# facebookresearch/DRTK

Measured on AMD Instinct MI355X. Metric: Mpixels/sec fwd+bwd, 100k-tri @ 2048x2048, 1/2/4/8 GPU; HBM BW %, higher is better.
Workload: dtype f32; 1 GPU; 8 views/GPU x 1 GPU, 100k-tri UV-sphere head mesh (F=100352, V=50400), 2048x2048, C=16 attribute channels, transform+rasterize+render+interpolate+mask+edge_grad_estimator+loss fwd+bwd; views_per_gpu=8, triangles=100352, vertices=50400, height=2048, width=2048, channels=16, grad_reset=set_to_none, parallelism=single GPU

## Files before the change

drtk_amd/capi.py:

```python
import ctypes
import os
from typing import Optional, Tuple

import torch as th

from drtk_amd.utils import native_library_paths

_lib = None

DRTK_F32, DRTK_F64 = 0, 1


_lib_path = None

_POISON = os.environ.get("DRTK_CAPI_POISON", "") not in ("", "0")


_GUARD = int(os.environ.get("DRTK_CAPI_GUARD", "0") or 0)
_guards = []


def _sentinel(dtype):
    return 0x5A if dtype == th.uint8 else (-7.25 if dtype.is_floating_point else -(2 ** 29) - 3)


def _out(*shape, dtype, device):
    if _GUARD:
        n = 1
        for d in shape:
            n *= int(d)
        g = _GUARD * (16 if dtype == th.uint8 else 1)
        flat = th.full((n + 2 * g,), _sentinel(dtype), dtype=dtype, device=device)
        _guards.append((flat, g, n))
        t = flat[g:g + n].view(*shape)
    else:
        t = th.empty(*shape, dtype=dtype, device=device)
    if _POISON and t.numel():
        if t.dtype.is_floating_point:
            t.fill_(float("nan"))
        elif t.dtype == th.uint8:
            t.fill_(0xA5)
        else:
            t.fill_(-(2 ** 30) - 7)
    return t


def check_guards() -> int:
    th.cuda.synchronize()
    k = len(_guards)
    for flat, g, n in _guards:
        s = _sentinel(flat.dtype)
        ok = bool((flat[:g] == s).all()) and bool((flat[g + n:] == s).all())
        if not ok:
            _guards.clear()
            raise AssertionError(f"a kernel wrote outside a {flat.dtype} output / workspace of {n} elements")
    _guards.clear()
    return k



def use_profiling_library(path: str) -> None:
    global _lib_path
    assert _lib is None, "the C-ABI library is already loaded"
    _lib_path = path


DEPTH_ORDERS = {"strict": 0, "fastmath": 1}


def use_depth_order(order: str) -> None:
    assert order in DEPTH_ORDERS, order
    _check(lib().drtk_amd_set_depth_order(DEPTH_ORDERS[order]), "set_depth_order")


def depth_order() -> str:
    o = lib().drtk_amd_get_depth_order()
    return next(k for k, v in DEPTH_ORDERS.items() if v == o)


def lib() -> ctypes.CDLL:
    global _lib
    if _lib is None:
        path = _lib_path or native_library_paths()[0]
        if not os.path.isfile(path):
            build_py = os.path.join(os.path.dirname(os.path.abspath(__file__)), "build.py")
            raise ImportError(f"{path} is missing: run `python {build_py}`")
        L = ctypes.CDLL(path)
        L.drtk_amd_status_string.restype = ctypes.c_char_p
        L.drtk_amd_status_string.argtypes = [ctypes.c_int]
        L.drtk_amd_version.restype = ctypes.c_char_p
        for name in EXPORTS:
            if name not in ("drtk_amd_status_string", "drtk_amd_version"):
                getattr(L, name).restype = ctypes.c_int
        _lib = L
    return _lib


EXPORTS = [
    "drtk_amd_status_string",
    "drtk_amd_version",
    "drtk_amd_set_depth_order",
    "drtk_amd_get_depth_order",
    "drtk_amd_rasterize_workspace_bytes",
    "drtk_amd_rasterize_lines_workspace_bytes",
    "drtk_amd_rasterize",
    "drtk_amd_rasterize_layers_workspace_bytes",
    "drtk_amd_rasterize_layers",
    "drtk_amd_render",
    "drtk_amd_render_backward",
    "drtk_amd_interpolate",
    "drtk_amd_interpolate_masked",
    "drtk_amd_interpolate_backward",
    "drtk_amd_interpolate_backward_workspace_bytes",
    "drtk_amd_interpolate_backward_ws",
    "drtk_amd_edge_grad_backward_workspace_bytes",
    "drtk_amd_edge_grad_backward",
    "drtk_amd_edge_grad_backward_fused_workspace_bytes",
    "drtk_amd_edge_grad_backward_fused",
    "drtk_amd_interpolation_matrix",
    "drtk_amd_interpolation_matrix_backward",
    "drtk_amd_interpolation_normal_matrix_values",
    "drtk_amd_interpolation_normal_matrix_values_backward",
    "drtk_amd_mipmap_grid_sampler_2d",
    "drtk_amd_mipmap_grid_sampler_2d_backward",
    "drtk_amd_grid_scatter_2d",
    "drtk_amd_grid_scatter_2d_backward",
    "drtk_amd_screen_space_uv_derivative",
    "drtk_amd_transform_pinhole",
    "drtk_amd_transform_pinhole_backward",
    "drtk_amd_geometry_face_forward",
    "drtk_amd_geometry_face_backward",
    "drtk_amd_geometry_face_gather",
    "drtk_amd_geometry_vertex_gather_workspace_bytes",
    "drtk_amd_geometry_vertex_gather",
    "drtk_amd_selftest_exact_div",
    "drtk_amd_kernel_timing_begin",
    "drtk_amd_kernel_timing_report",
]


class DrtkAmdError(RuntimeError):
    pass


def _check(status: int, what: str):
    if status != 0:
        raise DrtkAmdError(f"{what}: {lib().drtk_amd_status_string(status).decode()} (status {status})")


def _dt(t: th.Tensor) -> int:
    if t.dtype == th.float32:
        return DRTK_F32
    if t.dtype == th.float64:
        return DRTK_F64
    raise TypeError(f"drtk_amd: unsupported dtype {t.dtype}")


def _p(t: Optional[th.Tensor]):
    return ctypes.c_void_p(0 if t is None else t.data_ptr())


def _i(x) -> ctypes.c_int64:
    return ctypes.c_int64(int(x))


def _on_tensor_device(fn):
    import functools

    def tensors(args):
        for a in args:
            if isinstance(a, th.Tensor):
                yield a
            elif isinstance(a, (list, tuple)):
                yield from (x for x in a if isinstance(x, th.Tensor))

    @functools.wraps(fn)
    def guarded(*args, **kwargs):
        ts = list(tensors(list(args) + list(kwargs.values())))
        if not ts:
            return fn(*args, **kwargs)
        if not ts[0].is_cuda:
            raise DrtkAmdError("drtk_amd implements the MI355X (HIP) path only; got a CPU tensor")
        devs = {t.device for t in ts}
        if len(devs) != 1:
            raise DrtkAmdError(f"drtk_amd: tensors of one call on different devices: {sorted(map(str, devs))}")
        with th.cuda.device(ts[0].device):
            return fn(*args, **kwargs)

    return guarded


def _stream(t: th.Tensor, stream) -> ctypes.c_void_p:
    if not t.is_cuda:
        raise DrtkAmdError("drtk_amd implements the MI355X (HIP) path only; got a CPU tensor")
    s = th.cuda.current_stream(t.device) if stream is None else stream
    return ctypes.c_void_p(s.cuda_stream)


def _vi(vi: th.Tensor, n: int):
    assert vi.dtype == th.int32
    if vi.ndim == 2:
        c = vi.contiguous()
        return c, 0, c.shape[0]
    if vi.shape[0] > 1 and vi.stride(0) == 0:
        c = vi[0].contiguous()
        return c, 0, c.shape[0]
    c = vi.contiguous()
    return c, c.shape[1] * 3, c.shape[1]


def rasterize_workspace_bytes(N, F, H, W) -> int:
    out = ctypes.c_size_t(0)
    _check(lib().drtk_amd_rasterize_workspace_bytes(_i(N), _i(F), _i(H), _i(W), ctypes.byref(out)), "rasterize")
    return out.value


def rasterize_lines_workspace_bytes(N, H, W) -> int:
    out = ctypes.c_size_t(0)
    _check(lib().drtk_amd_rasterize_lines_workspace_bytes(_i(N), _i(H), _i(W), ctypes.byref(out)), "rasterize")
    return out.value


@_on_tensor_device
def rasterize(v, vi, height, width, stream=None, workspace=None, wireframe=False, out=None) -> Tuple[th.Tensor, th.Tensor]:
    v = v.contiguous()
    N, V, _ = v.shape
    vi_c, vi_sN, F = _vi(vi, N)
    if out is not None:
        depth, index = out
        assert depth.shape == (N, height, width) and index.shape == (N, height, width) and depth.is_contiguous() and index.is_contiguous()
        assert depth.dtype == th.float32 and index.dtype == th.int32
    else:
        depth = _out(N, height, width, dtype=th.float32, device=v.device)
        index = _out(N, height, width, dtype=th.int32, device=v.device)
    nbytes = rasterize_lines_workspace_bytes(N, height, width) if wireframe else rasterize_workspace_bytes(N, F, height, width)
    ws = workspace if workspace is not None else _out(nbytes, dtype=th.uint8, device=v.device)
    _check(
        lib().drtk_amd_rasterize(
            ctypes.c_int(_dt(v)), _p(v), _p(vi_c), _i(N), _i(V), _i(F), _i(vi_sN), _i(height), _i(width),
            ctypes.c_int(1 if wireframe else 0), _p(depth), _p(index), _p(ws), ctypes.c_size_t(ws.numel()),
            _stream(v, stream)),
        "rasterize")
    return depth, index


MAX_RASTER_LAYERS = 8


def rasterize_layers_workspace_bytes(N, F, H, W, num_layers) -> int:
    out = ctypes.c_size_t(0)
    _check(
        lib().drtk_amd_rasterize_layers_workspace_bytes(_i(N), _i(F), _i(H), _i(W), ctypes.c_int(int(num_layers)), ctypes.byref(out)),
        "rasterize_layers")
    return out.value


@_on_tensor_device
def rasterize_layers(v, vi, height, width, num_layers, stream=None, workspace=None, out=None) -> Tuple[th.Tensor, th.Tensor]:
    v = v.contiguous()
    N, V, _ = v.shape
    K = int(num_layers)
    vi_c, vi_sN, F = _vi(vi, N)
    nbytes = rasterize_layers_workspace_bytes(N, F, height, width, K)
    if out is not None:
        depth, index = out
        assert depth.shape == (N, K, height, width) and index.shape == (N, K, height, width) and depth.is_contiguous() and index.is_contiguous()
        assert depth.dtype == th.float32 and index.dtype == th.int32
    else:
        depth = _out(N, K, height, width, dtype=th.float32, device=v.device)
        index = _out(N, K, height, width, dtype=th.int32, device=v.device)
    ws = workspace if workspace is not None else _out(nbytes, dtype=th.uint8, device=v.device)
    _check(
        lib().drtk_amd_rasterize_layers(
            ctypes.c_int(_dt(v)), _p(v), _p(vi_c), _i(N), _i(V), _i(F), _i(vi_sN), _i(height), _i(width),
            ctypes.c_int(K), _p(depth), _p(index), _p(ws), ctypes.c_size_t(ws.numel()), _stream(v, stream)),
        "rasterize_layers")
    return depth, index


@_on_tensor_device
def render(v, vi, index_img, stream=None):
    v = v.contiguous()
    index_img = index_img.contiguous()
    N, V, _ = v.shape
    H, W = index_img.shape[1:]
    vi_c, vi_sN, F = _vi(vi, N)
    depth = _out(N, H, W, dtype=v.dtype, device=v.device)
    bary = _out(N, 3, H, W, dtype=v.dtype, device=v.device)
    _check(
        lib().drtk_amd_render(
            ctypes.c_int(_dt(v)), _p(v), _p(vi_c), _p(index_img), _i(N), _i(V), _i(F), _i(vi_sN), _i(H), _i(W),
            _p(depth), _p(bary), _stream(v, stream)),
        "render")
    return depth, bary


@_on_tensor_device
def render_backward(v, vi, index_img, grad_depth_img, grad_bary_img, stream=None):
    v = v.contiguous()
    index_img = index_img.contiguous()
    gd, gb = grad_depth_img.contiguous(), grad_bary_img.contiguous()
    N, V, _ = v.shape
    H, W = index_img.shape[1:]
    vi_c, vi_sN, F = _vi(vi, N)
    grad_v = _out(N, V, 3, dtype=v.dtype, device=v.device)
    _check(
        lib().drtk_amd_render_backward(
            ctypes.c_int(_dt(v)), _p(v), _p(vi_c), _p(index_img), _p(gd), _p(gb), _i(N), _i(V), _i(F), _i(vi_sN),
            _i(H), _i(W), _p(grad_v), _stream(v, stream)),
        "render_backward")
    return grad_v


@_on_tensor_device
def interpolate(attrs, vi, index_img, bary_img, stream=None, masked=False):
    attrs = attrs.contiguous()
    index_img = index_img.contiguous()
    bary_img = bary_img.contiguous()
    N, V, C = attrs.shape
    H, W = index_img.shape[1:]
    vi_c, vi_sN, F = _vi(vi, N)
    out = _out(N, C, H, W, dtype=attrs.dtype, device=attrs.device)
    fn = lib().drtk_amd_interpolate_masked if masked else lib().drtk_amd_interpolate
    _check(
        fn(ctypes.c_int(_dt(attrs)), _p(attrs), _p(vi_c), _p(index_img), _p(bary_img), _i(N), _i(V), _i(C), _i(F),
           _i(vi_sN), _i(H), _i(W), _p(out), _stream(attrs, stream)),
        "interpolate_masked" if masked else "interpolate")
    return out


def interpolate_masked(attrs, vi, index_img, bary_img, stream=None):
    return interpolate(attrs, vi, index_img, bary_img, stream, masked=True)


@_on_tensor_device
def interpolate_backward(grad_out, attrs, vi, index_img, bary_img, vert_requires_grad=True,
                         bary_requires_grad=True, stream=None, workspace=None):
    grad_out = grad_out.contiguous()
    attrs = attrs.contiguous()
    index_img = index_img.contiguous()
    bary_img = bary_img.contiguous()
    N, V, C = attrs.shape
    H, W = index_img.shape[1:]
    vi_c, vi_sN, F = _vi(vi, N)
    ag = _out(N, V, C, dtype=attrs.dtype, device=attrs.device) if vert_requires_grad else None
    bg = _out(N, 3, H, W, dtype=attrs.dtype, device=attrs.device) if bary_requires_grad else None
    ws, nbytes = None, 0
    if os.environ.get("DRTK_CAPI_NO_INTERP_WS"):
        workspace = False
    if vert_requires_grad and workspace is not False:
        out = ctypes.c_size_t(0)
        _check(lib().drtk_amd_interpolate_backward_workspace_bytes(ctypes.c_int(_dt(attrs)), _i(N), _i(V), _i(C), ctypes.byref(out)), "interpolate_backward")
        nbytes = int(out.value)
        if nbytes:
            ws = _out((nbytes + 3) // 4, dtype=th.float32, device=attrs.device)
            assert ws.data_ptr() % 64 == 0 or os.environ.get("DRTK_CAPI_GUARD"), "torch allocations are 256-byte aligned"
            if ws.data_ptr() % 64 != 0:
                ws, nbytes = None, 0
    _check(
        lib().drtk_amd_interpolate_backward_ws(
            ctypes.c_int(_dt(attrs)), _p(grad_out), _p(attrs), _p(vi_c), _p(index_img), _p(bary_img), _i(N), _i(V),
            _i(C), _i(F), _i(vi_sN), _i(H), _i(W), _p(ag), _p(bg), _p(ws), ctypes.c_size_t(nbytes), _stream(attrs, stream)),
        "interpolate_backward")
    return ag, bg


@_on_tensor_device
def interpolation_matrix(vi, index_img, bary_img, stream=None):
    index_img = index_img.contiguous()
    bary_img = bary_img.contiguous()
    N, H, W = index_img.shape
    vi_c, vi_sN, F = _vi(vi, N)
    row_pixels = th.nonzero(index_img.reshape(-1).ne(-1)).reshape(-1)
    R = row_pixels.numel()
    crow = th.arange(0, 3 * R + 1, 3, dtype=th.int64, device=index_img.device)
    col = _out(3 * R, dtype=th.int64, device=index_img.device)
    values = _out(3 * R, dtype=bary_img.dtype, device=bary_img.device)
    _check(
        lib().drtk_amd_interpolation_matrix(
            ctypes.c_int(_dt(bary_img)), _p(vi_c), _p(index_img), _p(bary_img), _p(row_pixels), _i(R), _i(N), _i(F),
            _i(vi_sN), _i(H), _i(W), _p(col), _p(values), _stream(bary_img, stream)),
        "interpolation_matrix")
    return crow, col, values, row_pixels


@_on_tensor_device
def interpolation_matrix_backward(grad_values, vi, index_img, row_pixels, stream=None):
    grad_values = grad_values.contiguous()
    index_img = index_img.contiguous()
    row_pixels = row_pixels.contiguous()
    N, H, W = index_img.shape
    vi_c, vi_sN, F = _vi(vi, N)
    bg = _out(N, 3, H, W, dtype=grad_values.dtype, device=grad_values.device)
    _check(
        lib().drtk_amd_interpolation_matrix_backward(
            ctypes.c_int(_dt(grad_values)), _p(grad_values), _p(vi_c), _p(index_img), _p(row_pixels),
            _i(row_pixels.numel()), _i(N), _i(F), _i(vi_sN), _i(H), _i(W), _p(bg), _stream(grad_values, stream)),
        "interpolation_matrix_backward")
    return bg


def _pairs(pair_indices, N):
    assert pair_indices.dtype == th.int32 and pair_indices.shape[-1] == 9
    if pair_indices.ndim == 2:
        return pair_indices.contiguous(), 0, pair_indices.shape[0]
    if pair_indices.shape[0] == N and N > 1 and pair_indices.stride(0) == 0:
        return pair_indices[0].contiguous(), 0, pair_indices.shape[1]
    p = pair_indices.contiguous()
    return p, p.shape[1] * 9, p.shape[1]


@_on_tensor_device
def interpolation_normal_matrix_values(pair_indices, index_img, bary_img, nnz, stream=None):
    index_img = index_img.contiguous()
    bary_img = bary_img.contiguous()
    N, H, W = index_img.shape
    pr, pair_sN, F = _pairs(pair_indices, N)
    values = _out(nnz, dtype=bary_img.dtype, device=bary_img.device)
    _check(
        lib().drtk_amd_interpolation_normal_matrix_values(
            ctypes.c_int(_dt(bary_img)), _p(pr), _p(index_img), _p(bary_img), _i(N), _i(F), _i(pair_sN), _i(H), _i(W),
            _i(nnz), _p(values), _stream(bary_img, stream)),
        "interpolation_normal_matrix_values")
    return values


@_on_tensor_device
def interpolation_normal_matrix_values_backward(grad_values, pair_indices, index_img, bary_img, stream=None):
    grad_values = grad_values.contiguous()
    index_img = index_img.contiguous()
    bary_img = bary_img.contiguous()
    N, H, W = index_img.shape
    pr, pair_sN, F = _pairs(pair_indices, N)
    bg = _out(N, 3, H, W, dtype=bary_img.dtype, device=bary_img.device)
    _check(
        lib().drtk_amd_interpolation_normal_matrix_values_backward(
            ctypes.c_int(_dt(bary_img)), _p(grad_values), _p(pr), _p(index_img), _p(bary_img), _i(N), _i(F),
            _i(pair_sN), _i(H), _i(W), _p(bg), _stream(bary_img, stream)),
        "interpolation_normal_matrix_values_backward")
    return bg


def _level_table(levels):
    lv = []
    for t in levels:
        ok = t.dim() == 4 and (t.shape[0] == 0 or t[0].is_contiguous()) and (t.stride(0) == 0 or t.stride(0) >= t[0].numel() or t.shape[0] <= 1)
        lv.append(t if ok else t.contiguous())
    n = len(lv)
    ptrs = (ctypes.c_void_p * n)(*[t.data_ptr() for t in lv])
    lh = (ctypes.c_int64 * n)(*[t.shape[2] for t in lv])
    lw = (ctypes.c_int64 * n)(*[t.shape[3] for t in lv])
    lsn = (ctypes.c_int64 * n)(*[(t.stride(0) if t.shape[0] > 1 else t.shape[1] * t.shape[2] * t.shape[3]) for t in lv])
    return lv, ptrs, lh, lw, lsn


def _grid_layout(grid):
    N, H, W, two = grid.shape
    sN, sH, sW, sC = grid.stride()
    P = H * W
    rows_ok = H <= 1 or sH == W * sW
    pixel_major = sC == 1 and sW == 2 and rows_ok and (N <= 1 or sN >= 2 * P)
    channel_major = sW == 1 and sC >= P and rows_ok and (N <= 1 or sN >= sC + P)
    if not (two == 2 and P > 0 and (pixel_major or channel_major)):
        grid = grid.contiguous()
        sN, sW, sC = 2 * P, 2, 1
    return grid, (ctypes.c_int64 * 3)(sN if N > 1 else 2 * P, sW, sC)


@_on_tensor_device
def mipmap_grid_sampler_2d(levels, grid, vt_dxdy_img, max_aniso, padding_mode=0, interpolation_mode=0,
                           align_corners=False, force_max_aniso=False, clip_grad=False, stream=None):
    lv, ptrs, lh, lw, lsn = _level_table(levels)
    grid, glayout = _grid_layout(grid)
    vt = vt_dxdy_img.contiguous()
    N, C = lv[0].shape[:2]
    H, W = grid.shape[1:3]
    out = _out(N, C, H, W, dtype=lv[0].dtype, device=lv[0].device)
    _check(
        lib().drtk_amd_mipmap_grid_sampler_2d(
            ctypes.c_int(_dt(lv[0])), ptrs, lh, lw, lsn, ctypes.c_int(len(lv)), _p(grid), glayout, _p(vt), _i(N), _i(C), _i(H), _i(W),
            ctypes.c_int(max_aniso), ctypes.c_int(padding_mode), ctypes.c_int(interpolation_mode),
            ctypes.c_int(bool(align_corners)), ctypes.c_int(bool(force_max_aniso)), ctypes.c_int(bool(clip_grad)),
            _p(out), _stream(lv[0], stream)),
        "mipmap_grid_sampler_2d")
    return out


@_on_tensor_device
def mipmap_grid_sampler_2d_backward(grad_out, levels, grid, vt_dxdy_img, max_aniso, padding_mode=0,
                                    interpolation_mode=0, align_corners=False, force_max_aniso=False,
                                    clip_grad=False, stream=None):
    lv, ptrs, lh, lw, lsn = _level_table(levels)
    grid, glayout = _grid_layout(grid)
    vt = vt_dxdy_img.contiguous()
    grad_out = grad_out.contiguous()
    N, C = lv[0].shape[:2]
    H, W = grid.shape[1:3]
    flat = _out(sum(t.numel() for t in lv), dtype=lv[0].dtype, device=lv[0].device)
    glv, off = [], 0
    for t in lv:
        glv.append(flat[off:off + t.numel()].view(t.shape))
        off += t.numel()
    gptrs = (ctypes.c_void_p * len(lv))(*[t.data_ptr() for t in glv])
    ggrid = th.empty_strided(grid.shape, grid.stride(), dtype=grid.dtype, device=grid.device)
    _check(
        lib().drtk_amd_mipmap_grid_sampler_2d_backward(
            ctypes.c_int(_dt(lv[0])), _p(grad_out), ptrs, lh, lw, lsn, ctypes.c_int(len(lv)), _p(grid), glayout, _p(vt), _i(N), _i(C),
            _i(H), _i(W), ctypes.c_int(max_aniso), ctypes.c_int(padding_mode), ctypes.c_int(interpolation_mode),
            ctypes.c_int(bool(align_corners)), ctypes.c_int(bool(force_max_aniso)), ctypes.c_int(bool(clip_grad)),
            gptrs, _p(ggrid), glayout, _stream(lv[0], stream)),
        "mipmap_grid_sampler_2d_backward")
    return glv, ggrid


@_on_tensor_device
def grid_scatter_2d(input, grid, output_height, output_width, padding_mode=1, interpolation_mode=0, align_corners=False,
                    stream=None, route_counts=None):
    input = input.contiguous()
    grid, glayout = _grid_layout(grid)
    N, C, H, W = input.shape
    assert grid.shape == (N, H, W, 2) and grid.dtype == input.dtype, (grid.shape, input.shape)
    if route_counts is not None:
        assert route_counts.numel() == 2 and route_counts.element_size() == 4 and route_counts.is_contiguous() and route_counts.device == input.device
    out = _out(N, C, int(output_height), int(output_width), dtype=input.dtype, device=input.device)
    _check(
        lib().drtk_amd_grid_scatter_2d(
            ctypes.c_int(_dt(input)), _p(input), _p(grid), glayout, _i(N), _i(C), _i(H), _i(W), _i(output_height),
            _i(output_width), ctypes.c_int(padding_mode), ctypes.c_int(interpolation_mode), ctypes.c_int(bool(align_corners)),
            _p(out), _p(route_counts), _stream(input, stream)),
        "grid_scatter_2d")
    return out


@_on_tensor_device
def grid_scatter_2d_backward(grad_out, input, grid, padding_mode=1, interpolation_mode=0, align_corners=False,
                             input_requires_grad=True, grid_requires_grad=True, stream=None):
    input = input.contiguous()
    grad_out = grad_out.contiguous()
    grid, glayout = _grid_layout(grid)
    N, C, H, W = input.shape
    OH, OW = grad_out.shape[2:]
    assert grad_out.shape[:2] == (N, C) and grid.shape == (N, H, W, 2)
    gi = _out(N, C, H, W, dtype=input.dtype, device=input.device) if input_requires_grad else None
    gg = None
    if grid_requires_grad:
        gg = th.empty_strided(grid.shape, grid.stride(), dtype=grid.dtype, device=grid.device)
        if _POISON and gg.numel():
            gg.fill_(float("nan"))
    _check(
        lib().drtk_amd_grid_scatter_2d_backward(
            ctypes.c_int(_dt(input)), _p(grad_out), _p(input), _p(grid), glayout, _i(N), _i(C), _i(H), _i(W), _i(OH), _i(OW),
            ctypes.c_int(padding_mode), ctypes.c_int(interpolation_mode), ctypes.c_int(bool(align_corners)), _p(gi), _p(gg),
            glayout, _stream(input, stream)),
        "grid_scatter_2d_backward")
    return gi, gg


@_on_tensor_device
def screen_space_uv_derivative(v, vt, vi, vti, index_img, bary_img, mask, campos, camrot, focal, stream=None):
    index_img = index_img.contiguous()
    bary_img = bary_img.contiguous()
    N, H, W = index_img.shape
    v_c, vt_c = v.contiguous(), vt.contiguous()
    v_sN = 0 if v_c.ndim == 2 else v_c.shape[1] * 3
    vt_sN = 0 if vt_c.ndim == 2 else vt_c.shape[1] * 2
    V, T = v_c.shape[-2], vt_c.shape[-2]
    vi_c, vti_c = vi.contiguous(), vti.contiguous()
    m = None if mask is None else mask.to(th.uint8).contiguous()
    out = _out(N, H, W, 2, 2, dtype=bary_img.dtype, device=bary_img.device)
    _check(
        lib().drtk_amd_screen_space_uv_derivative(
            ctypes.c_int(_dt(bary_img)), _p(v_c), _i(v_sN), _p(vt_c), _i(vt_sN), _p(vi_c), _p(vti_c), _p(index_img),
            _p(bary_img), _p(m), _p(campos.contiguous()), _p(camrot.contiguous()), _p(focal.contiguous()), _i(N), _i(V),
            _i(T), _i(vi_c.shape[0]), _i(H), _i(W), _p(out), _stream(bary_img, stream)),
        "screen_space_uv_derivative")
    return out


GEOMETRY_CHUNK = 256


def vertex_incidence_numpy(vi, num_vertices: int, chunk: int = GEOMETRY_CHUNK):
    import numpy as np

    t = np.asarray(vi, dtype=np.int64)
    t = t[None] if t.ndim == 2 else t
    B, F = t.shape[0], t.shape[1]
    V = int(num_vertices)
    keys = (t + (np.arange(B, dtype=np.int64) * V)[:, None, None]).reshape(-1)
    perm = np.argsort(keys, kind="stable")
    entries = (perm % max(3 * F, 1)).astype(np.int32)
    crow = np.searchsorted(keys[perm], np.arange(B * V + 1), side="left").astype(np.int64)
    length = np.diff(crow)
    nch = np.where(length > chunk, (length + chunk - 1) // chunk, 0)
    chunk_ptr = np.concatenate([[0], np.cumsum(nch)]).astype(np.int64)
    chunk_row = np.repeat(np.arange(B * V), nch)
    chunk_begin = crow[chunk_row] + (np.arange(len(chunk_row)) - chunk_ptr[chunk_row]) * chunk
    return tuple(a.astype(np.int32) for a in (crow, entries, chunk_ptr, chunk_begin, chunk_row))


def _geometry_topology(vi: th.Tensor):
    assert vi.dtype == th.int32
    c = vi.contiguous()
    if c.ndim == 2 or c.shape[0] == 1:
        return c, 0, 1
    return c, c.shape[1] * 3, c.shape[0]


@_on_tensor_device
def geometry_face_forward(v, vi, vt=None, vti=None, outputs=("normals", "areas", "edges"), stream=None):
    v = v.contiguous()
    N, V = v.shape[0], v.shape[1]
    vi_c, vi_sN, _ = _geometry_topology(vi)
    F = vi_c.shape[-2]
    shapes = {"normals": (N, F, 3), "areas": (N, F, 1), "edges": (N, F, 3, 3), "dpdt": (N, F, 2, 3),
              "dpdt_u": (N, F, 3), "v012": (N, F, 3, 3)}
    out = {k: _out(*shapes[k], dtype=v.dtype, device=v.device) for k in outputs}
    vt_c = None if vt is None else vt.contiguous()
    vti_c = None if vti is None else vti.contiguous()
    T = 0 if vt_c is None else vt_c.shape[1]
    _check(
        lib().drtk_amd_geometry_face_forward(
            ctypes.c_int(_dt(v)), _p(v), _i(V * 3), _p(vi_c), _i(vi_sN), _p(vt_c), _i(T * 2), _p(vti_c), _i(N), _i(V),
            _i(T), _i(F), *(_p(out.get(k)) for k in ("normals", "areas", "edges", "dpdt", "dpdt_u", "v012")),
            _stream(v, stream)),
        "geometry_face_forward")
    return out


@_on_tensor_device
def geometry_face_backward(v, vi, vt=None, vti=None, grad_vert=None, vert_sums=None, grad_normals=None,
                           grad_areas=None, grad_edges=None, grad_dpdt=None, grad_v012=None, stream=None):
    v = v.contiguous()
    N, V = v.shape[0], v.shape[1]
    vi_c, vi_sN, _ = _geometry_topology(vi)
    F = vi_c.shape[-2]
    vt_c = None if vt is None else vt.contiguous()
    vti_c = None if vti is None else vti.contiguous()
    T = 0 if vt_c is None else vt_c.shape[1]
    pos = _out(N, F, 3, 3, dtype=v.dtype, device=v.device)
    uv = None if vt_c is None else _out(N, F, 3, 2, dtype=v.dtype, device=v.device)
    c = [None if g is None else g.contiguous() for g in (grad_vert, vert_sums, grad_normals, grad_areas, grad_edges,
                                                          grad_dpdt, grad_v012)]
    _check(
        lib().drtk_amd_geometry_face_backward(
            ctypes.c_int(_dt(v)), _p(v), _i(V * 3), _p(vi_c), _i(vi_sN), _p(vt_c), _i(T * 2), _p(vti_c), _i(N), _i(V),
            _i(T), _i(F), *(_p(g) for g in c), _p(pos), _p(uv), _stream(v, stream)),
        "geometry_face_backward")
    return pos, uv


@_on_tensor_device
def geometry_face_gather(grad_vert, vi, num_faces=None, vert_sums=None, stream=None):
    g = grad_vert.contiguous()
    N, V, A = g.shape
    vi_c, vi_sN, _ = _geometry_topology(vi)
    F = vi_c.shape[-2]
    out = _out(N, F, A, dtype=g.dtype, device=g.device)
    s = None if vert_sums is None else vert_sums.contiguous()
    _check(lib().drtk_amd_geometry_face_gather(ctypes.c_int(_dt(g)), _p(g), _p(s), _p(vi_c), _i(vi_sN), _i(N), _i(V),
                                               _i(F), _i(A), _p(out), _stream(g, stream)),
           "geometry_face_gather")
    return out


@_on_tensor_device
def geometry_vertex_gather(src, incidence, num_vertices, per_corner=False, normalize=False, stream=None):
    src = src.contiguous()
    N, F, A = src.shape[0], src.shape[1], src.shape[-1]
    inc = [th.as_tensor(a, dtype=th.int32, device=src.device).contiguous() for a in incidence]
    crow, entries, chunk_ptr, chunk_begin, chunk_row = inc
    V = int(num_vertices)
    B = (crow.numel() - 1) // V if V else 1
    C = chunk_row.numel()
    out = _out(N, V, A, dtype=src.dtype, device=src.device)
    sums = _out(N, V, 3, dtype=src.dtype, device=src.device) if normalize else None
    need = ctypes.c_size_t(0)
    _check(lib().drtk_amd_geometry_vertex_gather_workspace_bytes(ctypes.c_int(_dt(src)), _i(N), _i(B), _i(C), _i(A),
                                                                 ctypes.byref(need)), "geometry_vertex_gather")
    ws = _out(max(need.value, 1), dtype=th.uint8, device=src.device)
    _check(
        lib().drtk_amd_geometry_vertex_gather(
            ctypes.c_int(_dt(src)), _p(src), _i(F * A * (3 if per_corner else 1)), ctypes.c_int(int(bool(per_corner))),
            _i(A), _p(crow), _p(entries), _p(chunk_ptr if C else None), _p(chunk_begin if C else None),
            _p(chunk_row if C else None), _i(C), _i(B), _i(N), _i(V), _i(F), ctypes.c_int(int(bool(normalize))), _p(out),
            _p(sums), _p(ws), ctypes.c_size_t(need.value), _stream(src, stream)),
        "geometry_vertex_gather")
    return out, sums


def edge_grad_backward_workspace_bytes(dtype, N, H, W) -> int:
    out = ctypes.c_size_t(0)
    code = DRTK_F32 if dtype == th.float32 else DRTK_F64
    _check(lib().drtk_amd_edge_grad_backward_workspace_bytes(ctypes.c_int(code), _i(N), _i(H), _i(W), ctypes.byref(out)),
           "edge_grad_backward")
    return out.value


@_on_tensor_device
def edge_grad_backward(v_pix, img, index_img, vi, grad_output, max_dp_dr=1e4, stream=None, workspace=None):
    v_pix = v_pix.contiguous()
    img = img.contiguous()
    index_img = index_img.contiguous()
    grad_output = grad_output.contiguous()
    N, V, _ = v_pix.shape
    C, H, W = img.shape[1:]
    vi_c, vi_sN, F = _vi(vi, N)
    out = _out(N, 3, H, W, dtype=v_pix.dtype, device=v_pix.device)
    nbytes = edge_grad_backward_workspace_bytes(v_pix.dtype, N, H, W)
    ws = workspace if workspace is not None else _out(nbytes, dtype=th.uint8, device=v_pix.device)
    _check(
        lib().drtk_amd_edge_grad_backward(
            ctypes.c_int(_dt(v_pix)), _p(v_pix), _p(img), _p(index_img), _p(vi_c), _p(grad_output), _i(N), _i(V),
            _i(C), _i(F), _i(vi_sN), _i(H), _i(W), ctypes.c_double(max_dp_dr), _p(out), _p(ws),
            ctypes.c_size_t(ws.numel()), _stream(v_pix, stream)),
        "edge_grad_backward")
    return out


@_on_tensor_device
def edge_grad_backward_fused(v_pix, img, index_img, vi, bary_img, grad_output, max_dp_dr=1e4, stream=None):
    v_pix = v_pix.contiguous()
    img = img.contiguous()
    index_img = index_img.contiguous()
    bary_img = bary_img.contiguous()
    grad_output = grad_output.contiguous()
    N, V, _ = v_pix.shape
    C, H, W = img.shape[1:]
    vi_c, vi_sN, F = _vi(vi, N)
    out = _out(N, V, 3, dtype=v_pix.dtype, device=v_pix.device)
    nb = ctypes.c_size_t(0)
    code = DRTK_F32 if v_pix.dtype == th.float32 else DRTK_F64
    _check(lib().drtk_amd_edge_grad_backward_fused_workspace_bytes(ctypes.c_int(code), _i(N), _i(H), _i(W), ctypes.byref(nb)),
           "edge_grad_backward_fused")
    ws = _out(nb.value, dtype=th.uint8, device=v_pix.device)
    _check(
        lib().drtk_amd_edge_grad_backward_fused(
            ctypes.c_int(_dt(v_pix)), _p(v_pix), _p(img), _p(index_img), _p(vi_c), _p(bary_img), _p(grad_output),
            _i(N), _i(V), _i(C), _i(F), _i(vi_sN), _i(H), _i(W), ctypes.c_double(max_dp_dr), _p(out), _p(ws),
            ctypes.c_size_t(ws.numel()), _stream(v_pix, stream)),
        "edge_grad_backward_fused")
    return out


def selftest_exact_div(dtype=th.float32, seed=1, count=1 << 28, device="cuda:0") -> int:
    out = th.zeros(1, dtype=th.int64, device=device)
    code = DRTK_F32 if dtype == th.float32 else DRTK_F64
    _check(lib().drtk_amd_selftest_exact_div(ctypes.c_int(code), ctypes.c_uint64(seed), _i(count), _p(out),
                                             _stream(out, None)), "selftest_exact_div")
    return int(out.item())


def kernel_timing_begin() -> None:
    _check(lib().drtk_amd_kernel_timing_begin(), "kernel_timing_begin")


def kernel_timing_report() -> dict:
    need = ctypes.c_size_t(0)
    buf = ctypes.create_string_buffer(1 << 16)
    _check(lib().drtk_amd_kernel_timing_report(buf, ctypes.c_size_t(len(buf)), ctypes.byref(need)), "kernel_timing_report")
    out = {}
    for line in buf.value.decode().splitlines():
        name, count, ms = line.rsplit("\t", 2)
        out[name.strip("()")] = (int(count), float(ms))
    return out
```

drtk_amd/csrc/rasterize.hip:

```cpp
#include <algorithm>

#include "common.hpp"
#include "segscatter.hpp"

#ifdef DRTK_AMD_ABLATION
namespace drtk_amd {
__device__ unsigned long long g_phase_clocks[16];
}
extern "C" __attribute__((visibility("default"))) int drtk_amd_debug_read_phases(unsigned long long* out) {
  if (hipDeviceSynchronize() != hipSuccess) return DRTK_ERR_LAUNCH;
  if (hipMemcpyFromSymbol(out, HIP_SYMBOL(drtk_amd::g_phase_clocks), 16 * sizeof(unsigned long long)) != hipSuccess) return DRTK_ERR_LAUNCH;
  const unsigned long long zero[16] = {};
  if (hipMemcpyToSymbol(HIP_SYMBOL(drtk_amd::g_phase_clocks), zero, sizeof(zero)) != hipSuccess) return DRTK_ERR_LAUNCH;
  return DRTK_OK;
}
#define DRTK_PHASE_INIT() unsigned long long drtk_phase_t_ = __builtin_readcyclecounter()
#define DRTK_PHASE(i)                                                     \
  do {                                                                    \
    if (DRTK_DBG(dbg, 256)) {  \
      const unsigned long long now_ = __builtin_readcyclecounter();       \
      atomicAdd(&::drtk_amd::g_phase_clocks[i], now_ - drtk_phase_t_);    \
      drtk_phase_t_ = __builtin_readcyclecounter();                       \
    }                                                                     \
  } while (0)
#else
#define DRTK_PHASE_INIT() do { } while (0)
#define DRTK_PHASE(i) do { } while (0)
#endif

namespace drtk_amd {
namespace {

constexpr uint32_t kCulled = 0xFFFFFFFFu;
constexpr uint32_t kFacingBit = 0x80000000u;
constexpr int kMaxSmallTiles = 4;

template <typename T>
struct TriSetup {
  T p0x, p0y, p1x, p1y, p2x, p2y;
  T dinv0, dinv1, dinv2;
  T sign_denom, abs_denom, rdenom;
  int bb_min_x, bb_min_y, bb_max_x, bb_max_y;
  bool c0, c1, c2;
  bool tl0, tl1, tl2;
  uint32_t z_lo_bits;
};

template <typename T>
struct DivRange;
template <>
struct DivRange<float> {
  static __device__ constexpr float lo() { return 0x1p-60f; }
  static __device__ constexpr float hi() { return 0x1p60f; }
  static __device__ constexpr float tiny() { return 0x1p-100f; }
};
template <>
struct DivRange<double> {
  static __device__ constexpr double lo() { return 0x1p-500; }
  static __device__ constexpr double hi() { return 0x1p500; }
  static __device__ constexpr double tiny() { return 0x1p-900; }
};
__device__ __forceinline__ float fma_t(float a, float b, float c) {
  return __builtin_fmaf(a, b, c);
}
__device__ __forceinline__ double fma_t(double a, double b, double c) {
  return __builtin_fma(a, b, c);
}
template <typename T>
__device__ __forceinline__ bool exact_div_ok(T d) {
  return d >= DivRange<T>::lo() && d <= DivRange<T>::hi();
}
template <typename T>
__device__ __forceinline__ T exact_div(T n, T d, T r, bool range_ok) {
  const T q0 = n * r;
  if (range_ok && (q0 >= DivRange<T>::tiny() || n == T(0))) {
    const T q1 = fma_t(fma_t(-d, q0, n), r, q0);
    return fma_t(fma_t(-d, q1, n), r, q1);
  }
  return n / d;
}

template <typename T>
__device__ __forceinline__ T markstein2(T n, T d, T r, T q0) {
  const T q1 = fma_t(fma_t(-d, q0, n), r, q0);
  return fma_t(fma_t(-d, q1, n), r, q1);
}

__device__ __forceinline__ float exact_rcp(float x) {
  const uint32_t bits = __float_as_uint(x);
  const float ax = __uint_as_float(bits & 0x7FFFFFFFu);
  if ((bits & 0x7FFFFFu) != 0x7FFFFFu && ax >= 0x1p-100f && ax <= 0x1p100f) {
    const float y = __builtin_amdgcn_rcpf(x);
    return __builtin_fmaf(y, __builtin_fmaf(-x, y, 1.0f), y);
  }
  return 1.0f / x;
}
__device__ __forceinline__ double exact_rcp(double x) {
  return 1.0 / x;
}
__device__ __forceinline__ bool fast_rcp_ok(float x) {
  const uint32_t bits = __float_as_uint(x);
  const float ax = __uint_as_float(bits & 0x7FFFFFFFu);
  return ((bits & 0x7FFFFFu) != 0x7FFFFFu) & (ax >= 0x1p-100f) & (ax <= 0x1p100f);
}
__device__ __forceinline__ float fast_rcp(float x) {
  const float y = __builtin_amdgcn_rcpf(x);
  return __builtin_fmaf(y, __builtin_fmaf(-x, y, 1.0f), y);
}
__device__ __forceinline__ bool fast_rcp_ok(double) {
  return true;
}
__device__ __forceinline__ bool fast_rcp_ok_clamped(float x) {
  const uint32_t bits = __float_as_uint(x);
  return ((bits & 0x7FFFFFu) != 0x7FFFFFu) & (__uint_as_float(bits & 0x7FFFFFFFu) <= 0x1p100f);
}
__device__ __forceinline__ bool fast_rcp_ok_clamped(double) {
  return true;
}
template <typename T>
__device__ __forceinline__ T smallest_positive_if(bool on);
template <>
__device__ __forceinline__ float smallest_positive_if<float>(bool on) {
  return __uint_as_float(on ? 1u : 0u);
}
template <>
__device__ __forceinline__ double smallest_positive_if<double>(bool on) {
  return __longlong_as_double(on ? 1ll : 0ll);
}
__device__ __forceinline__ double fast_rcp(double x) {
  return 1.0 / x;
}

template <typename T>
__device__ __forceinline__ uint32_t z_lower_bound_bits(T min_x, T max_x, T min_y, T max_y, T abs_denom, T zmin) {
  const T ext = (max_x - min_x > max_y - min_y ? max_x - min_x : max_y - min_y) + T(2);
  const T eps = sizeof(T) == 4 ? T(5.97e-8) : T(1.12e-16);
  const T delta = T(40) * eps * ext * ext / abs_denom + T(2e-6);
  if (!(delta < T(0.25))) return 0u;
  const T cap = (T(1) / Eps<T>::value()) * (T(1) - T(2e-6));
  const T zb = zmin * (T(1) - delta);
  const float lo = static_cast<float>(zb < cap ? zb : cap);
  const uint32_t bits = __float_as_uint(lo);
  return (lo > 0.0f && bits > 8u) ? bits - 8u : 0u;
}

template <typename T>
__device__ __forceinline__ uint32_t z_upper_bound_bits(const TriSetup<T>& s) {
  const T min_x = min3(s.p0x, s.p1x, s.p2x), min_y = min3(s.p0y, s.p1y, s.p2y);
  const T max_x = max3(s.p0x, s.p1x, s.p2x), max_y = max3(s.p0y, s.p1y, s.p2y);
  const T ext = (max_x - min_x > max_y - min_y ? max_x - min_x : max_y - min_y) + T(2);
  const T eps = sizeof(T) == 4 ? T(5.97e-8) : T(1.12e-16);
  const T delta = T(40) * eps * ext * ext / s.abs_denom + T(2e-6);
  if (!(delta < T(0.25))) return 0xFFFFFFFFu;
  const T zb = (T(1) / min3(s.dinv0, s.dinv1, s.dinv2)) / (T(1) - delta);
  const float hi = static_cast<float>(zb);
  if (!(hi > 0.0f && hi < 1e30f)) return 0xFFFFFFFFu;
  return __float_as_uint(hi) + 8u;
}

template <typename T>
__device__ __forceinline__ bool tri_bbox(
    const T* __restrict__ v_n, const int32_t* __restrict__ vi_face, int H, int W, int& bx0,
    int& by0, int& bx1, int& by1, bool& positive, float& z_mean, uint32_t& z_lo_bits) {
  const int32_t vi_0 = static_cast<int32_t>(static_cast<uint32_t>(vi_face[0]) & 0x0FFFFFFFu);
  const int32_t vi_1 = vi_face[1];
  const int32_t vi_2 = vi_face[2];
  if (vi_0 == vi_1 && vi_1 == vi_2) return false;
  const T p0x = v_n[3 * (int64_t)vi_0 + 0], p0y = v_n[3 * (int64_t)vi_0 + 1], p0z = v_n[3 * (int64_t)vi_0 + 2];
  const T p1x = v_n[3 * (int64_t)vi_1 + 0], p1y = v_n[3 * (int64_t)vi_1 + 1], p1z = v_n[3 * (int64_t)vi_1 + 2];
  const T p2x = v_n[3 * (int64_t)vi_2 + 0], p2y = v_n[3 * (int64_t)vi_2 + 1], p2z = v_n[3 * (int64_t)vi_2 + 2];
  if (!(p0z > T(1e-8f) && p1z > T(1e-8f) && p2z > T(1e-8f))) return false;
  const T min_x = min3(p0x, p1x, p2x), min_y = min3(p0y, p1y, p2y);
  const T max_x = max3(p0x, p1x, p2x), max_y = max3(p0y, p1y, p2y);
  if (!(min_x <= T(W - 1) && min_y <= T(H - 1) && max_x > T(0) && max_y > T(0))) return false;
  const T v01x = p1x - p0x, v01y = p1y - p0y, v02x = p2x - p0x, v02y = p2y - p0y;
  const T den = v01x * v02y - v01y * v02x;
  if (den == T(0)) return false;
  positive = den > T(0);
  z_lo_bits = z_lower_bound_bits<T>(min_x, max_x, min_y, max_y, den > T(0) ? den : -den, min3(p0z, p1z, p2z));
  z_mean = static_cast<float>((p0z + p1z + p2z) * T(1.0 / 3.0));
  bx0 = max(0, trunc_i32(min_x));
  by0 = max(0, trunc_i32(min_y));
  bx1 = min(W - 1, static_cast<int32_t>(static_cast<uint32_t>(trunc_i32(max_x)) + 1u));
  by1 = min(H - 1, static_cast<int32_t>(static_cast<uint32_t>(trunc_i32(max_y)) + 1u));
  return bx0 <= bx1 && by0 <= by1;
}

template <typename T>
__device__ __forceinline__ bool tri_setup(
    const T* __restrict__ v_n, const int32_t* __restrict__ vi_face, int H, int W, TriSetup<T>& s) {
  const int32_t vi_0 = static_cast<int32_t>(static_cast<uint32_t>(vi_face[0]) & 0x0FFFFFFFu);
  const int32_t vi_1 = vi_face[1];
  const int32_t vi_2 = vi_face[2];
  if (vi_0 == vi_1 && vi_1 == vi_2) return false;
  s.p0x = v_n[3 * (int64_t)vi_0 + 0];
  s.p0y = v_n[3 * (int64_t)vi_0 + 1];
  s.p1x = v_n[3 * (int64_t)vi_1 + 0];
  s.p1y = v_n[3 * (int64_t)vi_1 + 1];
  s.p2x = v_n[3 * (int64_t)vi_2 + 0];
  s.p2y = v_n[3 * (int64_t)vi_2 + 1];
  const T p0z = v_n[3 * (int64_t)vi_0 + 2];
  const T p1z = v_n[3 * (int64_t)vi_1 + 2];
  const T p2z = v_n[3 * (int64_t)vi_2 + 2];
  if (!(p0z > T(1e-8f) && p1z > T(1e-8f) && p2z > T(1e-8f))) return false;
  const T min_x = min3(s.p0x, s.p1x, s.p2x), min_y = min3(s.p0y, s.p1y, s.p2y);
  const T max_x = max3(s.p0x, s.p1x, s.p2x), max_y = max3(s.p0y, s.p1y, s.p2y);
  if (!(min_x <= T(W - 1) && min_y <= T(H - 1) && max_x > T(0) && max_y > T(0))) return false;
  const T v01x = s.p1x - s.p0x, v01y = s.p1y - s.p0y;
  const T v02x = s.p2x - s.p0x, v02y = s.p2y - s.p0y;
  const T v12x = s.p2x - s.p1x, v12y = s.p2y - s.p1y;
  const T den = v01x * v02y - v01y * v02x;
  if (den == T(0)) return false;
  s.sign_denom = den > T(0) ? T(1) : T(-1);
  s.abs_denom = den > T(0) ? den : -den;
  s.rdenom = T(1) / s.abs_denom;
  s.bb_min_x = max(0, trunc_i32(min_x));
  s.bb_min_y = max(0, trunc_i32(min_y));
  s.bb_max_x = min(W - 1, static_cast<int32_t>(static_cast<uint32_t>(trunc_i32(max_x)) + 1u));
  s.bb_max_y = min(H - 1, static_cast<int32_t>(static_cast<uint32_t>(trunc_i32(max_y)) + 1u));
  s.dinv0 = T(1) / epsclamp(p0z);
  s.dinv1 = T(1) / epsclamp(p1z);
  s.dinv2 = T(1) / epsclamp(p2z);
  s.c0 = vi_1 <= vi_2;
  s.c1 = vi_2 <= vi_0;
  s.c2 = vi_0 <= vi_1;
  const bool pos = den > T(0);
  s.tl0 = pos ? (v12y < T(0) || (v12y == T(0) && v12x > T(0))) : (v12y > T(0) || (v12y == T(0) && v12x < T(0)));
  s.tl1 = pos ? (v02y > T(0) || (v02y == T(0) && v02x < T(0))) : (v02y < T(0) || (v02y == T(0) && v02x > T(0)));
  s.tl2 = pos ? (v01y < T(0) || (v01y == T(0) && v01x > T(0))) : (v01y > T(0) || (v01y == T(0) && v01x < T(0)));
  s.z_lo_bits = 0;
  return true;
}

template <typename T>
__device__ __forceinline__ T edge_fn(T ax, T ay, T bx, T by, T px, T py) {
  return (py - ay) * (bx - ax) - (px - ax) * (by - ay);
}
template <typename T>
__device__ __forceinline__ T canon_edge(bool a_le_b, T ax, T ay, T bx, T by, T px, T py) {
  return a_le_b ? edge_fn(ax, ay, bx, by, px, py) : -edge_fn(bx, by, ax, ay, px, py);
}

template <typename T>
__device__ __forceinline__ bool fragment(const TriSetup<T>& s, int x, int y, uint32_t& depth_bits) {
  const T px = static_cast<T>(x), py = static_cast<T>(y);
  T b0 = canon_edge(s.c0, s.p1x, s.p1y, s.p2x, s.p2y, px, py) * s.sign_denom;
  T b1 = canon_edge(s.c1, s.p2x, s.p2y, s.p0x, s.p0y, px, py) * s.sign_denom;
  T b2 = canon_edge(s.c2, s.p0x, s.p0y, s.p1x, s.p1y, px, py) * s.sign_denom;
  if (!((b0 >= T(0)) && (b1 >= T(0)) && (b2 >= T(0)))) return false;
  if ((!s.tl0 && b0 == T(0)) || (!s.tl1 && b1 == T(0)) || (!s.tl2 && b2 == T(0))) return false;
  b0 /= s.abs_denom;
  b1 /= s.abs_denom;
  b2 /= s.abs_denom;
  const T depth_inverse = s.dinv0 * b0 + s.dinv1 * b1 + s.dinv2 * b2;
  const float depth = static_cast<float>(T(1) / epsclamp(depth_inverse));
  depth_bits = __float_as_uint(depth);
  return true;
}

#ifndef DRTK_RASTER_QUEUE_SHARDS
#define DRTK_RASTER_QUEUE_SHARDS 8
#endif
constexpr int kQueueShards = DRTK_RASTER_QUEUE_SHARDS;
constexpr int kQueueStride = 32;
constexpr uint32_t kItemEmpty = 0x80000000u;

struct BinLayout {
  int tile_shift;
  int tiles_x, tiles_y;
  int64_t tiles_per_view, num_tiles;
  size_t off_count, off_cursor, off_big_count, off_view_stats, off_queue, zero_bytes;
  size_t off_offset, off_range, off_pre, off_big_list, off_pairs, off_items, total_bytes;
  int64_t max_items;
};

constexpr int kSplit4Min = 384, kSplit4Max = 2048;
inline int split_threshold(int64_t N, int64_t F) {
#ifndef DRTK_RASTER_SPLIT_SLOTS
#define DRTK_RASTER_SPLIT_SLOTS 4
#endif
  const int64_t slots = int64_t(num_compute_units()) * DRTK_RASTER_SPLIT_SLOTS;
  const int64_t t = (N * F * 13) / (20 * (slots > 0 ? slots : 1));
  return static_cast<int>(t < kSplit4Min ? kSplit4Min : (t > kSplit4Max ? kSplit4Max : t));
}
__host__ __device__ inline uint32_t make_item(uint32_t tile, uint32_t sub, uint32_t split_log) {
  return tile | (sub << 24) | (split_log << 28);
}

inline size_t align_up(size_t x, size_t a) {
  return (x + a - 1) / a * a;
}

inline BinLayout make_layout(int64_t N, int64_t F, int64_t H, int64_t W) {
  BinLayout L;
  const int64_t t64 = N * ceil_div(W, 64) * ceil_div(H, 64);
  L.tile_shift = (t64 >= 2048) ? 6 : 5;
  const int64_t ts = int64_t(1) << L.tile_shift;
  L.tiles_x = static_cast<int>(ceil_div(W, ts));
  L.tiles_y = static_cast<int>(ceil_div(H, ts));
  L.tiles_per_view = int64_t(L.tiles_x) * L.tiles_y;
  L.num_tiles = N * L.tiles_per_view;
  size_t o = 0;
  L.off_count = o;
  o += align_up(sizeof(unsigned long long) * L.num_tiles, 256);
  L.off_cursor = o;
  o += align_up(sizeof(unsigned long long) * L.num_tiles, 256);
  L.off_big_count = o;
  o += align_up(sizeof(int32_t) * (N > 0 ? N : 1), 256);
  L.off_view_stats = o;
  o += align_up(sizeof(float) * 4 * (N > 0 ? N : 1), 256);
  L.off_queue = o;
  o += align_up(sizeof(int32_t) * kQueueStride * (1 + kQueueShards), 256);
  L.zero_bytes = o;
  L.off_offset = o;
  o += align_up(sizeof(int32_t) * (L.num_tiles + 1), 256);
  L.off_range = o;
  o += align_up(sizeof(uint2) * N * F, 256);
  L.off_pre = o;
  o += align_up(sizeof(uint4) * N * F, 256);
  L.off_big_list = o;
  o += align_up(sizeof(int32_t) * N * F, 256);
  L.off_pairs = o;
  o += align_up(sizeof(int32_t) * kMaxSmallTiles * N * F, 256);
  L.max_items = L.num_tiles + 16 * ((kMaxSmallTiles * N * F) / kSplit4Min);
  L.off_items = o;
  o += align_up(sizeof(uint32_t) * L.max_items, 256);
  L.total_bytes = o > 0 ? o : 256;
  return L;
}

template <bool BOTH, bool FETCH>
__device__ __forceinline__ int wave_agg_inc2(unsigned long long* __restrict__ counters, int key, bool on, bool hi) {
  const int lane = lane_id();
  unsigned long long todo = __ballot(on);
  int pos = 0;
  while (todo) {
    const int leader = __builtin_amdgcn_readfirstlane(__builtin_ctzll(todo));
    const int k = __builtin_amdgcn_readlane(key, leader);
    const bool mine = on && key == k;
    const unsigned long long same = __ballot(mine);
    const unsigned long long same_hi = __ballot(mine && hi);
    const unsigned long long same_lo = BOTH ? same : (same & ~same_hi);
    unsigned long long base = 0;
    if (lane == leader) {
      const unsigned long long add =
          static_cast<unsigned long long>(__popcll(same_lo)) | (static_cast<unsigned long long>(__popcll(same_hi)) << 32);
      if (FETCH) {
        base = atomicAdd(counters + k, add);
      } else {
        atomicAdd(counters + k, add);
      }
    }
    if (FETCH) {
      const unsigned lo = __builtin_amdgcn_readlane(static_cast<int>(base & 0xFFFFFFFFull), leader);
      const unsigned hh = __builtin_amdgcn_readlane(static_cast<int>(base >> 32), leader);
      const unsigned long long below = (1ull << lane) - 1ull;
      if (mine) pos = hi ? static_cast<int>(hh) + __popcll(same_hi & below) : static_cast<int>(lo) + __popcll(same_lo & below);
    }
    todo &= ~same;
  }
  return pos;
}

template <typename T>
__global__ __launch_bounds__(kBlock) void bin_count_kernel(
    const T* __restrict__ v, const int32_t* __restrict__ vi, int F, int64_t V, int64_t vi_sN, int H,
    int W, int tile_shift, int tiles_x, int tiles_per_view, unsigned long long* __restrict__ tile_count,
    int32_t* __restrict__ big_count, int32_t* __restrict__ big_list,
    uint2* __restrict__ tri_range, uint4* __restrict__ tri_pre, float* __restrict__ view_stats) {
  const int n = blockIdx.y;
  const int f = blockIdx.x * kBlock + threadIdx.x;
  const bool in_range = f < F;
  int bx0, by0, bx1, by1;
  uint2 r = make_uint2(kCulled, kCulled);
  int tx0 = 0, ty0 = 0, tw = 0, ntiles = 0;
  bool positive = false;
  float z_mean = 0.0f;
  uint32_t z_lo_bits = 0;
  if (in_range &&
      tri_bbox<T>(v + int64_t(n) * V * 3, vi + int64_t(n) * vi_sN + int64_t(f) * 3, H, W, bx0, by0, bx1, by1, positive, z_mean, z_lo_bits)) {
    const bool fits = bx1 < 65536 && by1 < 65536;
    tri_pre[int64_t(n) * F + f] = make_uint4(
        static_cast<uint32_t>(bx0) | (static_cast<uint32_t>(bx1) << 16), static_cast<uint32_t>(by0) | (static_cast<uint32_t>(by1) << 16),
        fits ? z_lo_bits : 0u, fits ? 1u : 0u);
    tx0 = bx0 >> tile_shift;
    ty0 = by0 >> tile_shift;
    const int tx1 = bx1 >> tile_shift, ty1 = by1 >> tile_shift;
    r.x = static_cast<uint32_t>(tx0) | (static_cast<uint32_t>(tx1) << 16);
    r.y = static_cast<uint32_t>(ty0) | (static_cast<uint32_t>(ty1) << 16) | (positive ? kFacingBit : 0u);
    tw = tx1 - tx0 + 1;
    ntiles = tw * (ty1 - ty0 + 1);
  }
  if ((blockIdx.x & 63) == 0) {
    const bool live = ntiles >= 1;
    float zp = (live && positive) ? z_mean : 0.0f, zn = (live && !positive) ? z_mean : 0.0f;
#pragma unroll
    for (int o = 32; o > 0; o >>= 1) {
      zp += __shfl_xor(zp, o);
      zn += __shfl_xor(zn, o);
    }
    const int cp = __popcll(__ballot(live && positive)), cn = __popcll(__ballot(live && !positive));
    if (lane_id() == 0 && (cp | cn)) {
      float* st = view_stats + 4 * n;
      if (cp) {
        atomic_add_global(st + 0, zp);
        atomic_add_global(st + 1, static_cast<float>(cp));
      }
      if (cn) {
        atomic_add_global(st + 2, zn);
        atomic_add_global(st + 3, static_cast<float>(cn));
      }
    }
  }
  if (in_range) tri_range[int64_t(n) * F + f] = r;
  const bool small = ntiles >= 1 && ntiles <= kMaxSmallTiles;
  const int base = n * tiles_per_view;
  for (int s = 0; s < kMaxSmallTiles; ++s) {
    const bool on = small && s < ntiles;
    const int dy = on ? s / tw : 0;
    const int dx = on ? s - dy * tw : 0;
    const int t = base + (ty0 + dy) * tiles_x + tx0 + dx;
    wave_agg_inc2<true, false>(tile_count, t, on, positive);
  }
  const bool big = ntiles > kMaxSmallTiles;
  if (__ballot(big)) {
    const int pos = wave_agg_inc<true>(big_count, n, big);
    if (big) big_list[int64_t(n) * F + pos] = f;
  }
}

__global__ __launch_bounds__(1024) void bin_scan_kernel(
    const unsigned long long* __restrict__ tile_count64, int32_t* __restrict__ tile_offset, int num_tiles,
    int tile_shift, int split4, uint32_t* __restrict__ items, int32_t* __restrict__ queue) {
  constexpr int kThreads = 1024, kWaves = kThreads / kWave, kVals = 5, kReg = 8;
  __shared__ int32_t s_wave[kWaves][kVals];
  const int tid = threadIdx.x, lane = tid & (kWave - 1), wave = tid / kWave;
  const int chunk = (num_tiles + kThreads - 1) / kThreads;
  const int begin = tid * chunk;
  const int end = min(begin + chunk, num_tiles);
  const int max_split_log = max(0, min(2, tile_shift - 4));
  auto split_log_of = [&](int c) {
    int sl = c > 4 * split4 ? 2 : (c > split4 ? 1 : 0);
    return min(sl, max_split_log);
  };
  auto class_of = [&](int c, int sl) { return c == 0 ? 3 : 2 - sl; };
  const bool in_regs = chunk <= kReg;
  int32_t cnt[kReg];
#pragma unroll
  for (int j = 0; j < kReg; ++j) {
    cnt[j] = (in_regs && begin + j < end) ? static_cast<int32_t>(tile_count64[begin + j] & 0xFFFFFFFFull) : 0;
  }
  auto count_at = [&](int j) -> int32_t {
    return static_cast<int32_t>(tile_count64[begin + j] & 0xFFFFFFFFull);
  };
  int32_t v[kVals] = {0, 0, 0, 0, 0};
  auto tally = [&](int c) {
    const int sl = split_log_of(c);
    v[0] += c;
    v[1 + class_of(c, sl)] += 1 << (2 * sl);
  };
  if (in_regs) {
#pragma unroll
    for (int j = 0; j < kReg; ++j) {
      if (begin + j < end) tally(cnt[j]);
    }
  } else {
    for (int j = 0; begin + j < end; ++j) tally(count_at(j));
  }
  int32_t inc[kVals];
#pragma unroll
  for (int k = 0; k < kVals; ++k) {
    int32_t x = v[k];
#pragma unroll
    for (int o = 1; o < kWave; o <<= 1) {
      const int32_t up = __shfl_up(x, o);
      if (lane >= o) x += up;
    }
    inc[k] = x;
    if (lane == kWave - 1) s_wave[wave][k] = x;
  }
  __syncthreads();
  int32_t before[kVals], total[kVals];
#pragma unroll
  for (int k = 0; k < kVals; ++k) {
    int32_t lo = 0, all = 0;
    for (int w = 0; w < kWaves; ++w) {
      const int32_t t = s_wave[w][k];
      all += t;
      if (w < wave) lo += t;
    }
    before[k] = lo + inc[k] - v[k];
    total[k] = all;
  }
  int32_t slot[4];
  {
    int32_t acc = 0;
#pragma unroll
    for (int k = 0; k < 4; ++k) {
      slot[k] = acc + before[1 + k];
      acc += total[1 + k];
    }
    if (tid == 0) {
      queue[1] = acc;
      tile_offset[num_tiles] = total[0];
    }
  }
  int32_t run = before[0];
  auto emit = [&](int i, int c) {
    tile_offset[i] = run;
    run += c;
    const int sl = split_log_of(c);
    const int cls = class_of(c, sl);
    const int n_sub = 1 << (2 * sl);
    for (int j = 0; j < n_sub; ++j) items[slot[cls] + j] = make_item(static_cast<uint32_t>(i), j, sl) | (c == 0 ? kItemEmpty : 0u);
    slot[cls] += n_sub;
  };
  if (in_regs) {
#pragma unroll
    for (int j = 0; j < kReg; ++j) {
      if (begin + j < end) emit(begin + j, cnt[j]);
    }
  } else {
    for (int j = 0; begin + j < end; ++j) emit(begin + j, count_at(j));
  }
}

__global__ __launch_bounds__(kBlock) void bin_fill_kernel(
    const uint2* __restrict__ tri_range, int F, int tiles_x, int tiles_per_view,
    const int32_t* __restrict__ tile_offset, unsigned long long* __restrict__ tile_cursor,
    int32_t* __restrict__ pairs) {
  const int n = blockIdx.y;
  const int f = blockIdx.x * kBlock + threadIdx.x;
  int tx0 = 0, ty0 = 0, tw = 0, ntiles = 0;
  bool positive = false;
  if (f < F) {
    const uint2 r = tri_range[int64_t(n) * F + f];
    if (r.x != kCulled) {
      tx0 = r.x & 0xFFFF;
      ty0 = r.y & 0xFFFF;
      tw = static_cast<int>(r.x >> 16) - tx0 + 1;
      ntiles = tw * (static_cast<int>((r.y & ~kFacingBit) >> 16) - ty0 + 1);
      positive = (r.y & kFacingBit) != 0;
    }
  }
  const bool small = ntiles >= 1 && ntiles <= kMaxSmallTiles;
  const int base = n * tiles_per_view;
  const int lane = lane_id();
  const unsigned long long below = (1ull << lane) - 1ull;
  int t_[kMaxSmallTiles], leader_[kMaxSmallTiles], rank_[kMaxSmallTiles];
  bool on_[kMaxSmallTiles];
  unsigned long long base_[kMaxSmallTiles];
#pragma unroll
  for (int s = 0; s < kMaxSmallTiles; ++s) {
    const bool on = small && s < ntiles;
    const int dy = on ? s / tw : 0;
    const int dx = on ? s - dy * tw : 0;
    const int t = base + (ty0 + dy) * tiles_x + tx0 + dx;
    int leader = lane, rank = 0;
    unsigned long long add = 0;
    unsigned long long todo = __ballot(on);
    while (todo) {
      const int ld = __builtin_amdgcn_readfirstlane(__builtin_ctzll(todo));
      const int k = __builtin_amdgcn_readlane(t, ld);
      const bool mine = on && t == k;
      const unsigned long long same = __ballot(mine);
      const unsigned long long same_neg = __ballot(mine && !positive);
      const unsigned long long same_pos = same & ~same_neg;
      if (mine) {
        leader = ld;
        rank = positive ? __popcll(same_pos & below) : __popcll(same_neg & below);
        add = static_cast<unsigned long long>(__popcll(same_pos)) | (static_cast<unsigned long long>(__popcll(same_neg)) << 32);
      }
      todo &= ~same;
    }
    on_[s] = on, t_[s] = t, leader_[s] = leader, rank_[s] = rank;
    base_[s] = 0;
    if (on && lane == leader) base_[s] = atomicAdd(tile_cursor + t, add);
  }
#pragma unroll
  for (int s = 0; s < kMaxSmallTiles; ++s) {
    const unsigned lo = __shfl(static_cast<unsigned>(base_[s] & 0xFFFFFFFFull), leader_[s]);
    const unsigned hi = __shfl(static_cast<unsigned>(base_[s] >> 32), leader_[s]);
    if (on_[s]) {
      const int pos = static_cast<int>(positive ? lo : hi) + rank_[s];
      pairs[positive ? tile_offset[t_[s]] + pos : tile_offset[t_[s] + 1] - 1 - pos] = f;
    }
  }
}


__device__ __forceinline__ int mbcnt(unsigned long long m) {
  return __builtin_amdgcn_mbcnt_hi(static_cast<uint32_t>(m >> 32), __builtin_amdgcn_mbcnt_lo(static_cast<uint32_t>(m), 0u));
}
template <int K>
__device__ __forceinline__ int row_bcast(int x) {
  return __builtin_amdgcn_mov_dpp(x, 0x150 + K, 0xF, 0xF, true);
}
template <int K>
__device__ __forceinline__ float row_bcast(float x) {
  return __builtin_bit_cast(float, row_bcast<K>(__builtin_bit_cast(int, x)));
}
template <int K>
__device__ __forceinline__ double row_bcast(double x) {
  const unsigned long long u = __builtin_bit_cast(unsigned long long, x);
  const unsigned lo = row_bcast<K>(static_cast<int>(u & 0xFFFFFFFFull));
  const unsigned hi = row_bcast<K>(static_cast<int>(u >> 32));
  return __builtin_bit_cast(double, (static_cast<unsigned long long>(hi) << 32) | lo);
}

template <typename T>
struct TriRow {
  T ax[3], ay[3], dx[3], dy[3];
  T abs_denom, rdenom, dinv0, dinv1, dinv2;
  int id_tl;
  int box;
  uint32_t z_lo;
};
constexpr int kTlShift = 29;
constexpr int kBoxDraw = 1 << 24;

template <int K, typename T>
__device__ __forceinline__ TriRow<T> row_bcast_tri(const TriRow<T>& o) {
  TriRow<T> u;
#pragma unroll
  for (int k = 0; k < 3; ++k) {
    u.ax[k] = row_bcast<K>(o.ax[k]);
    u.ay[k] = row_bcast<K>(o.ay[k]);
    u.dx[k] = row_bcast<K>(o.dx[k]);
    u.dy[k] = row_bcast<K>(o.dy[k]);
  }
  u.abs_denom = row_bcast<K>(o.abs_denom);
  u.rdenom = row_bcast<K>(o.rdenom);
  u.dinv0 = row_bcast<K>(o.dinv0);
  u.dinv1 = row_bcast<K>(o.dinv1);
  u.dinv2 = row_bcast<K>(o.dinv2);
  u.id_tl = row_bcast<K>(o.id_tl);
  u.box = row_bcast<K>(o.box);
  u.z_lo = static_cast<uint32_t>(row_bcast<K>(static_cast<int>(o.z_lo)));
  return u;
}

template <typename T>
__device__ __forceinline__ TriRow<T> make_row_state(bool valid, const TriSetup<T>& s, int f, uint32_t z_lo, int x0, int y0, int x1, int y1) {
  TriRow<T> o;
  o.z_lo = z_lo;
  const T px[3] = {s.p1x, s.p2x, s.p0x}, py[3] = {s.p1y, s.p2y, s.p0y};
  const T qx[3] = {s.p2x, s.p0x, s.p1x}, qy[3] = {s.p2y, s.p0y, s.p1y};
  const bool c[3] = {s.c0, s.c1, s.c2};
#pragma unroll
  for (int k = 0; k < 3; ++k) {
    o.ax[k] = c[k] ? px[k] : qx[k];
    o.ay[k] = c[k] ? py[k] : qy[k];
    const T bx = c[k] ? qx[k] : px[k], by = c[k] ? qy[k] : py[k];
    const bool neg = c[k] ? (s.sign_denom < T(0)) : !(s.sign_denom < T(0));
    const T ex = bx - o.ax[k], ey = by - o.ay[k];
    o.dx[k] = neg ? -ex : ex;
    o.dy[k] = neg ? -ey : ey;
  }
  o.abs_denom = s.abs_denom;
  o.rdenom = s.rdenom;
  o.dinv0 = s.dinv0;
  o.dinv1 = s.dinv1;
  o.dinv2 = s.dinv2;
  const int bx0 = max(s.bb_min_x, x0), bx1 = min(s.bb_max_x, x1);
  const int by0 = max(s.bb_min_y, y0), by1 = min(s.bb_max_y, y1);
  const bool draw = valid && bx0 <= bx1 && by0 <= by1;
  o.box = draw ? ((bx0 - x0) | ((by0 - y0) << 6) | ((bx1 - bx0) << 12) | ((by1 - by0) << 18) | kBoxDraw) : 0;
  o.id_tl = f | ((s.tl0 ? 1 : 0) | (s.tl1 ? 2 : 0) | (s.tl2 ? 4 : 0)) << kTlShift;
  return o;
}

template <typename T>
using TriOwn = TriRow<T>;

template <typename T, int TILE_SHIFT, bool EARLY_Z, bool FM, bool PEEL, int STRIDE = 16>
__device__ __forceinline__ void shade_rows(
    const TriRow<T>& u, float lane16_half, float x0f, float y0f, unsigned long long* __restrict__ zbuf,
    const unsigned long long* __restrict__ zthr, int dbg) {
  constexpr float kTileF = static_cast<float>(1 << TILE_SHIFT);
  const float rx0f = static_cast<float>(u.box & 63), ry0f = static_cast<float>((u.box >> 6) & 63);
  const float bwf = static_cast<float>(((u.box >> 12) & 63) + 1), bhf = static_cast<float>(((u.box >> 18) & 63) + 1);
  const float npxf = (u.box & kBoxDraw) ? bwf * bhf : 0.0f;
  const float bx0f = x0f + rx0f, by0f = y0f + ry0f;
  const float c0f = __builtin_fmaf(ry0f, kTileF, rx0f);
  float rbw = __builtin_amdgcn_rcpf(bwf);
  asm volatile("" : "+v"(rbw));
  const bool div_ok = exact_div_ok(u.abs_denom);
  const T thr0 = smallest_positive_if<T>(!(u.id_tl & (1 << kTlShift)));
  const T thr1 = smallest_positive_if<T>(!(u.id_tl & (2 << kTlShift)));
  const T thr2 = smallest_positive_if<T>(!(u.id_tl & (4 << kTlShift)));
  const T b_min = u.abs_denom * T(0x1p-40);
  const unsigned long long id = static_cast<uint32_t>(u.id_tl) & ((1u << kTlShift) - 1u);
#ifdef DRTK_AMD_ABLATION
  if (STRIDE == 16 && DRTK_DBG(dbg, 512)) {
    const int need = static_cast<int>((npxf + 15.0f) * 0.0625f);
    int mx = need;
#pragma unroll
    for (int o = 32; o >= 16; o >>= 1) mx = max(mx, __shfl_xor(mx, o));
    int sum = need;
#pragma unroll
    for (int o = 32; o >= 16; o >>= 1) sum += __shfl_xor(sum, o);
    if (lane_id() == 0) {
      atomicAdd(&::drtk_amd::g_phase_clocks[10], static_cast<unsigned long long>(mx));
      atomicAdd(&::drtk_amd::g_phase_clocks[11], static_cast<unsigned long long>(sum));
      atomicAdd(&::drtk_amd::g_phase_clocks[12], 1ull);
    }
  }
#endif
  for (float ph = lane16_half; ph < npxf; ph += static_cast<float>(STRIDE)) {
    const float fly = __builtin_truncf(ph * rbw);
    const float flx = __builtin_fmaf(-fly, bwf, ph - 0.5f);
    const T px = static_cast<T>(bx0f + flx), py = static_cast<T>(by0f + fly);
    const T b0 = (py - u.ay[0]) * u.dx[0] - (px - u.ax[0]) * u.dy[0];
    const T b1 = (py - u.ay[1]) * u.dx[1] - (px - u.ax[1]) * u.dy[1];
    const T b2 = (py - u.ay[2]) * u.dx[2] - (px - u.ax[2]) * u.dy[2];
    if (!((b0 >= thr0) & (b1 >= thr1) & (b2 >= thr2))) continue;
    const int zi = static_cast<int>(__builtin_fmaf(fly, kTileF, c0f) + flx);
    unsigned long long thr = 0;
    if constexpr (PEEL) {
      thr = zthr[zi];
      if (thr == ~0ull) continue;
      if (static_cast<uint32_t>(thr) == static_cast<uint32_t>(id)) continue;
    }
    if (EARLY_Z) {
      if (u.z_lo > static_cast<uint32_t>(zbuf[zi] >> 32)) continue;
    }
    if (DRTK_DBG(dbg, 4)) {
      atomicMin(&zbuf[zi], id);
      continue;
    }
    T d0 = T(0), d1 = T(0), d2 = T(0);
    if constexpr (!FM) {
      const T q0 = b0 * u.rdenom, q1 = b1 * u.rdenom, q2 = b2 * u.rdenom;
      const bool fast_ok = div_ok & (min3(b0, b1, b2) >= b_min);
      d0 = markstein2(b0, u.abs_denom, u.rdenom, q0);
      d1 = markstein2(b1, u.abs_denom, u.rdenom, q1);
      d2 = markstein2(b2, u.abs_denom, u.rdenom, q2);
      if (__ballot(!fast_ok) != 0) {
        d0 = exact_div(b0, u.abs_denom, u.rdenom, div_ok);
        d1 = exact_div(b1, u.abs_denom, u.rdenom, div_ok);
        d2 = exact_div(b2, u.abs_denom, u.rdenom, div_ok);
      }
    }
    const T depth_inverse = FM ? ((b1 * u.dinv1 + b0 * u.dinv0) + b2 * u.dinv2) * u.rdenom : u.dinv0 * d0 + u.dinv1 * d1 + u.dinv2 * d2;
    const T di = depth_inverse > Eps<T>::value() ? depth_inverse : Eps<T>::value();
    T rd = fast_rcp(di);
    if (__ballot(!fast_rcp_ok_clamped(di)) != 0) rd = exact_rcp(di);
    const float depth = static_cast<float>(rd);
    const unsigned long long packed = (static_cast<unsigned long long>(__float_as_uint(depth)) << 32) | id;
    if constexpr (PEEL) {
      if (!(packed > thr)) continue;
    }
    atomicMin(&zbuf[zi], packed);
  }
}

template <typename T, int TILE_SHIFT, bool EARLY_Z, bool FM, bool PEEL>
__device__ __forceinline__ void raster_rows(
    const TriOwn<T>& o, int nsteps, int x0, int y0, unsigned long long* __restrict__ zbuf,
    const unsigned long long* __restrict__ zthr, int dbg) {
  const float x0f = static_cast<float>(x0), y0f = static_cast<float>(y0);
  const float lane16_half = static_cast<float>(lane_id() & 15) + 0.5f;
  for (int k = 0; k < nsteps; ++k) {
    TriRow<T> u;
    switch (k) {
#define DRTK_ROW_STEP(K) case K: u = row_bcast_tri<K>(o); break;
      DRTK_ROW_STEP(0) DRTK_ROW_STEP(1) DRTK_ROW_STEP(2) DRTK_ROW_STEP(3) DRTK_ROW_STEP(4) DRTK_ROW_STEP(5)
      DRTK_ROW_STEP(6) DRTK_ROW_STEP(7) DRTK_ROW_STEP(8) DRTK_ROW_STEP(9) DRTK_ROW_STEP(10) DRTK_ROW_STEP(11)
      DRTK_ROW_STEP(12) DRTK_ROW_STEP(13) DRTK_ROW_STEP(14)
      default: u = row_bcast_tri<15>(o); break;
#undef DRTK_ROW_STEP
    }
    shade_rows<T, TILE_SHIFT, EARLY_Z, FM, PEEL>(u, lane16_half, x0f, y0f, zbuf, zthr, dbg);
  }
}

#ifndef DRTK_RASTER_WAVES_PER_SIMD
#define DRTK_RASTER_WAVES_PER_SIMD 6
#endif
#ifndef DRTK_RASTER_BLOCK
#define DRTK_RASTER_BLOCK 512
#endif
constexpr int kRasterBlock = DRTK_RASTER_BLOCK;
constexpr int kRasterWaves = kRasterBlock / kWave;
constexpr int kPlain = 0, kLayerFirst = 1, kLayerPeel = 2;
template <typename T, int MODE = kPlain>
constexpr int raster_waves_per_simd() {
  return sizeof(T) == 4 ? (MODE == kLayerPeel ? (DRTK_RASTER_WAVES_PER_SIMD < 4 ? DRTK_RASTER_WAVES_PER_SIMD : 4) : DRTK_RASTER_WAVES_PER_SIMD) : 2;
}
constexpr int kIdRing = 128;
#ifndef DRTK_RASTER_COOP_MIN
#define DRTK_RASTER_COOP_MIN 256
#endif
#ifndef DRTK_RASTER_COOP_MIN_DENSE
#define DRTK_RASTER_COOP_MIN_DENSE 1024
#endif
#ifndef DRTK_RASTER_COOP_DENSE
#define DRTK_RASTER_COOP_DENSE 64
#endif
constexpr int kCoopMin = DRTK_RASTER_COOP_MIN, kCoopMinDense = DRTK_RASTER_COOP_MIN_DENSE, kCoopDense = DRTK_RASTER_COOP_DENSE;
constexpr int kCoopBatch = 64;
constexpr int kCoopMax = 256;

template <typename T, int TILE_SHIFT, bool FM, int MODE>
__device__ __forceinline__ void tile_raster_body(
    const T* __restrict__ v, const int32_t* __restrict__ vi, int F, int64_t V, int64_t vi_sN,
    int H, int W, int tiles_x, int tiles_per_view, const int32_t* __restrict__ tile_offset,
    const unsigned long long* __restrict__ tile_count, const float* __restrict__ view_stats,
    const int32_t* __restrict__ pairs, const int32_t* __restrict__ big_count,
    const int32_t* __restrict__ big_list, const uint2* __restrict__ tri_range, const uint4* __restrict__ tri_pre,
    const uint32_t* __restrict__ items, int32_t* __restrict__ queue, float* __restrict__ depth_img,
    int32_t* __restrict__ index_img, int dbg, int num_layers, int layer) {
  constexpr int TILE = 1 << TILE_SHIFT;
  constexpr int NPIX = TILE * TILE;
  constexpr bool PEEL = MODE == kLayerPeel;
  __shared__ unsigned long long zbuf[NPIX];
  unsigned long long* zthr = nullptr;
  uint32_t* tmin = nullptr;
  if constexpr (PEEL) {
    __shared__ unsigned long long s_zthr[NPIX];
    __shared__ uint32_t s_tmin[(TILE / 8) * (TILE / 8)];
    zthr = s_zthr;
    tmin = s_tmin;
  }
  __shared__ uint32_t s_zmax[(TILE / 8) * (TILE / 8)];
  __shared__ int32_t s_idq[kRasterWaves][kIdRing];
  __shared__ int32_t s_idk[kRasterWaves][kIdRing];
  __shared__ int s_item;
  __shared__ int s_queue[3];
  __shared__ int32_t s_coop[kCoopMax];
  __shared__ int s_ncoop;
  constexpr int kTriWords = sizeof(TriRow<T>) / 4;
  static_assert(sizeof(TriRow<T>) % 4 == 0, "TriRow is parked in LDS word by word");
  __shared__ uint32_t s_tri[kCoopMin > 0 ? kCoopBatch * kTriWords : 1];
  static_assert(kCoopBatch % kRasterWaves == 0 && kCoopBatch / kRasterWaves <= kWave, "cooperative batch set-up needs kRasterWaves | kCoopBatch");
  static_assert(
      (sizeof(unsigned long long) * NPIX + sizeof(uint32_t) * (TILE / 8) * (TILE / 8) + 2 * sizeof(int32_t) * kRasterWaves * kIdRing +
       sizeof(int32_t) * kCoopMax + sizeof(uint32_t) * kCoopBatch * kTriWords + 64 +
       (PEEL ? sizeof(unsigned long long) * NPIX + sizeof(uint32_t) * (TILE / 8) * (TILE / 8) : 0)) *
              (raster_waves_per_simd<T, MODE>() * 4 / kRasterWaves > 0 ? raster_waves_per_simd<T, MODE>() * 4 / kRasterWaves : 1) <= 160 * 1024,
      "tile_raster's static LDS no longer fits the workgroups per CU its launch bounds ask for");

  const int tid = threadIdx.x;
  const int wave = __builtin_amdgcn_readfirstlane(tid / kWave), lane = tid & (kWave - 1);
  const int n_items = queue[1];
  auto pop = [&]() {
    int shard = s_queue[0], dry = s_queue[1], idx = -1;
    while (dry < kQueueShards) {
      idx = atomicAdd(&queue[kQueueStride * (1 + shard)], 1) * kQueueShards + shard;
      if (idx < n_items) break;
      idx = -1;
      ++dry;
      shard = (shard + 1) % kQueueShards;
    }
    s_queue[0] = shard, s_queue[1] = dry, s_queue[2] = idx;
  };
  if (tid == 0) {
    s_queue[0] = blockIdx.x % kQueueShards, s_queue[1] = 0;
    s_ncoop = 0;
    pop();
  }
  for (int i = tid; i < NPIX; i += kRasterBlock) zbuf[i] = ~0ull;
  DRTK_PHASE_INIT();
  for (;;) {
    if (tid == 0) s_item = s_queue[2];
    __syncthreads();
    if (tid == 0) DRTK_PHASE(0);
    const int item_index = s_item;
    if (item_index < 0) break;
    const uint32_t item = items[item_index];
    const int tile = item & 0xFFFFFF;
    const int sub = (item >> 24) & 0xF, split_log = (item >> 28) & 3;
    const int n = tile / tiles_per_view;
    const int t_in_view = tile - n * tiles_per_view;
    const int ty = t_in_view / tiles_x, tx = t_in_view - ty * tiles_x;
    const int ss = TILE >> split_log;
    const int x0 = (tx << TILE_SHIFT) + (sub & ((1 << split_log) - 1)) * ss;
    const int y0 = (ty << TILE_SHIFT) + (sub >> split_log) * ss;
    const int x1 = min(x0 + ss - 1, W - 1), y1 = min(y0 + ss - 1, H - 1);
    if (!(x0 < W && y0 < H)) {
      if (tid == 0) pop();
      __syncthreads();
      continue;
    }
    {
      const int rows = y1 - y0 + 1;
      const int nbig = big_count[n];
      int64_t img_base_of_item = int64_t(n) * H * W;
      if constexpr (MODE != kPlain) img_base_of_item = (int64_t(n) * num_layers + layer) * H * W;
      const int64_t img_base = img_base_of_item;
      const bool vec_ok = (W & 3) == 0;
      typedef int32_t IQuad __attribute__((ext_vector_type(4), aligned(4)));
      typedef float FQuad __attribute__((ext_vector_type(4), aligned(4)));
      const int quads_per_row = ss >> 2;
      bool exhausted = false;
      if constexpr (PEEL) {
        if (!((item & kItemEmpty) && nbig == 0)) {
          const int ss_log = TILE_SHIFT - split_log;
          const int64_t prev_base = img_base - int64_t(H) * W;
          int any = 0;
          typedef int32_t IQuadIn __attribute__((ext_vector_type(4), aligned(4)));
          typedef float FQuadIn __attribute__((ext_vector_type(4), aligned(4)));
          for (int q = tid; q < (ss << (ss_log - 2)); q += kRasterBlock) {
            const int row = q >> (ss_log - 2), col = (q & ((ss >> 2) - 1)) << 2;
            int32_t pi[4] = {-1, -1, -1, -1};
            float pd[4] = {0.0f, 0.0f, 0.0f, 0.0f};
            const int x = x0 + col;
            if (row < rows && x <= x1) {
              const int64_t o = prev_base + int64_t(y0 + row) * W + x;
              const bool whole = vec_ok || x + 3 <= x1;
              if (whole) {
                const IQuadIn iq = *reinterpret_cast<const IQuadIn*>(index_img + o);
                pi[0] = iq.x, pi[1] = iq.y, pi[2] = iq.z, pi[3] = iq.w;
              } else {
                for (int j = 0; j < 4 && x + j <= x1; ++j) pi[j] = index_img[o + j];
              }
              if ((pi[0] & pi[1] & pi[2] & pi[3]) >= 0) {
                any = 1;
                if (whole) {
                  const FQuadIn dq = *reinterpret_cast<const FQuadIn*>(depth_img + o);
                  pd[0] = dq.x, pd[1] = dq.y, pd[2] = dq.z, pd[3] = dq.w;
                } else {
                  for (int j = 0; j < 4 && x + j <= x1; ++j) pd[j] = depth_img[o + j];
                }
              }
            }
#pragma unroll
            for (int j = 0; j < 4; ++j) {
              zthr[(row << TILE_SHIFT) + col + j] =
                  pi[j] < 0 ? ~0ull : ((static_cast<unsigned long long>(__float_as_uint(pd[j])) << 32) | static_cast<uint32_t>(pi[j]));
            }
          }
          exhausted = __syncthreads_or(any) == 0;
          if (!exhausted) {
            const int nb_thr = ss >> 3;
            for (int by = wave; by < nb_thr; by += kRasterWaves) {
              uint32_t m = 0xFFFFFFFFu;
              if (lane < ss) {
#pragma unroll
                for (int r = 0; r < 8; ++r) m = min(m, static_cast<uint32_t>(zthr[(((by << 3) + r) << TILE_SHIFT) + lane] >> 32));
              }
              m = min(m, static_cast<uint32_t>(__builtin_amdgcn_mov_dpp(static_cast<int>(m), 0xB1, 0xF, 0xF, true)));
              m = min(m, static_cast<uint32_t>(__builtin_amdgcn_mov_dpp(static_cast<int>(m), 0x4E, 0xF, 0xF, true)));
              m = min(m, static_cast<uint32_t>(__builtin_amdgcn_mov_dpp(static_cast<int>(m), 0x141, 0xF, 0xF, true)));
              if ((lane & 7) == 0 && lane < ss) tmin[by * nb_thr + (lane >> 3)] = m;
            }
            __syncthreads();
          }
        }
      }
      if (((item & kItemEmpty) && nbig == 0) || exhausted) {
        for (int q = tid; q < rows * quads_per_row; q += kRasterBlock) {
          const int row = q / quads_per_row;
          const int col = (q - row * quads_per_row) << 2;
          const int y = y0 + row, x = x0 + col;
          if (x > x1) continue;
          const int64_t o = img_base + int64_t(y) * W + x;
          int none = -1;
          float zero = 0.0f;
          asm volatile("" : "+v"(none), "+v"(zero));
          if (vec_ok || x + 3 <= x1) {
            *reinterpret_cast<IQuad*>(index_img + o) = IQuad{none, none, none, none};
            *reinterpret_cast<FQuad*>(depth_img + o) = FQuad{zero, zero, zero, zero};
          } else {
            for (int j = 0; j < 4 && x + j <= x1; ++j) {
              index_img[o + j] = none;
              depth_img[o + j] = zero;
            }
          }
        }
        if (tid == 0) pop();
        __syncthreads();
        continue;
      }

      const T* v_n = v + int64_t(n) * V * 3;
      const int32_t* vi_n = vi + int64_t(n) * vi_sN;
      const int nb = ss >> 3;
      int32_t* idq = s_idq[wave];
      int32_t* idk = s_idk[wave];

      const int begin = tile_offset[tile], end_all = tile_offset[tile + 1];
      const int n_pos = static_cast<int>(tile_count[tile] >> 32);
      const float* st = view_stats + 4 * n;
      const bool pos_first = st[0] * st[3] <= st[2] * st[1];
      const uint4* pre_n = tri_pre + int64_t(n) * F;
      const int32_t* big_n = big_list + int64_t(n) * F;
      const uint2* range_n = tri_range + int64_t(n) * F;
      for (int phase = 0; phase < 2; ++phase) {
        if (phase == 1 && DRTK_DBG(dbg, 64)) break;
        const bool take_pos = (phase == 0) == pos_first;
        const int g_begin = take_pos ? begin : begin + n_pos, g_end = take_pos ? begin + n_pos : end_all;
        auto accept = [&](int bx_min, int by_min, int bx_max, int by_max, uint32_t z_lo_bits) -> bool {
          if (!(bx_min <= x1 && bx_max >= x0 && by_min <= y1 && by_max >= y0)) return false;
          if (phase == 0 || z_lo_bits == 0 || DRTK_DBG(dbg, 16)) return true;
          const int cx0 = (max(bx_min, x0) - x0) >> 3, cx1 = (min(bx_max, x1) - x0) >> 3;
          const int cy0 = (max(by_min, y0) - y0) >> 3, cy1 = (min(by_max, y1) - y0) >> 3;
          if ((cx1 - cx0 + 1) * (cy1 - cy0 + 1) > 16) return true;
          uint32_t far = 0;
          for (int by = cy0; by <= cy1; ++by)
            for (int bx = cx0; bx <= cx1; ++bx) far = max(far, s_zmax[by * nb + bx]);
          return !(z_lo_bits > far);
        };
        auto pre_accept = [&](int f, int& size) -> bool {
          const uint4 pre = pre_n[f];
          size = NPIX + 1;
          if (pre.w == 0u) return true;
          const int bx_min = static_cast<int>(pre.x & 0xFFFFu), by_min = static_cast<int>(pre.y & 0xFFFFu);
          const int bx_max = static_cast<int>(pre.x >> 16), by_max = static_cast<int>(pre.y >> 16);
          size = (min(bx_max, x1) - max(bx_min, x0) + 1) * (min(by_max, y1) - max(by_min, y0) + 1);
          return accept(bx_min, by_min, bx_max, by_max, pre.z);
        };
        const int per_wave = (g_end - g_begin + kRasterWaves - 1) / kRasterWaves;
        int cursor = g_begin + wave * per_wave;
        const int end = min(cursor + per_wave, g_end);
        const int big_per_wave = phase == 0 ? (nbig + kRasterWaves - 1) / kRasterWaves : 0;
        int big_cursor = wave * big_per_wave;
        const int big_end = min(big_cursor + big_per_wave, phase == 0 ? nbig : 0);
        int head = 0, tail = 0;
        const int coop_min = end_all - begin >= kCoopDense ? kCoopMinDense : kCoopMin;
        if (DRTK_DBG(dbg, 8)) cursor = end, big_cursor = big_end;
        for (;;) {
          while (tail - head < kWave && (cursor < end || big_cursor < big_end)) {
            bool ok = false;
            int f = 0, size = 0;
            if (cursor < end) {
              const int i = cursor + lane;
              if (i < end) {
                f = pairs[i];
                ok = pre_accept(f, size);
              }
              cursor += kWave;
            } else {
              const int i = big_cursor + lane;
              if (i < big_end) {
                f = big_n[i];
                const uint2 r = range_n[f];
                const int rtx0 = r.x & 0xFFFF, rtx1 = r.x >> 16, rty0 = r.y & 0xFFFF, rty1 = (r.y & ~kFacingBit) >> 16;
                ok = tx >= rtx0 && tx <= rtx1 && ty >= rty0 && ty <= rty1 && pre_accept(f, size);
              }
              big_cursor += kWave;
            }
            if (kCoopMin > 0) {
              const bool coop = ok && size >= coop_min && size <= NPIX;
              const unsigned long long mc = __ballot(coop);
              if (mc != 0) {
                const int leader = __builtin_ctzll(mc);
                int base = 0;
                if (lane == leader) base = atomicAdd(&s_ncoop, __popcll(mc));
                base = __shfl(base, leader);
                const int slot = base + mbcnt(mc);
                if (coop && slot < kCoopMax) {
                  s_coop[slot] = f;
                  ok = false;
                }
              }
            }
            const unsigned long long m = __ballot(ok);
            if (ok) {
              const int slot = (tail + mbcnt(m)) & (kIdRing - 1);
              idq[slot] = f;
              idk[slot] = size;
            }
            tail += __popcll(m);
          }
          const int cnt = min(kWave, tail - head);
          if (cnt == 0) break;
          wave_lds_sync();
          const int e = ((lane & 15) << 2) | (lane >> 4);
          bool valid = e < cnt;
          int f;
#ifndef DRTK_RASTER_NO_SORT
          if (cnt > 4) {
            const bool has = lane < cnt;
            const int slot = (head + lane) & (kIdRing - 1);
            const int f_nat = has ? idq[slot] : 0;
            uint32_t p = has ? ((static_cast<uint32_t>(idk[slot]) << 6) | static_cast<uint32_t>(lane)) : static_cast<uint32_t>(lane);
#pragma unroll
            for (int k = 2; k <= kWave; k <<= 1) {
#pragma unroll
              for (int j = k >> 1; j > 0; j >>= 1) {
                const uint32_t other = static_cast<uint32_t>(__shfl_xor(static_cast<int>(p), j));
                const bool take_max = ((lane & j) == 0) == ((lane & k) == 0);
                p = take_max ? max(p, other) : min(p, other);
              }
            }
            const int src = __shfl(static_cast<int>(p & 63u), e);
            f = __shfl(f_nat, src);
            if (!valid) f = 0;
          } else
#endif
          {
            f = valid ? idq[(head + e) & (kIdRing - 1)] : 0;
          }
          head += cnt;
          wave_lds_sync();
          TriSetup<T> s = {};
          uint32_t z_lo = 0;
          if (valid) {
            const uint4 pre = pre_n[f];
            z_lo = pre.z;
            valid = tri_setup<T>(v_n, vi_n + int64_t(f) * 3, H, W, s);
            if (valid && pre.w == 0u) valid = accept(s.bb_min_x, s.bb_min_y, s.bb_max_x, s.bb_max_y, 0u);
            if constexpr (PEEL) {
              if (valid) {
                const uint32_t z_hi = z_upper_bound_bits<T>(s);
                const int cx0 = (max(s.bb_min_x, x0) - x0) >> 3, cx1 = (min(s.bb_max_x, x1) - x0) >> 3;
                const int cy0 = (max(s.bb_min_y, y0) - y0) >> 3, cy1 = (min(s.bb_max_y, y1) - y0) >> 3;
                if (cx0 <= cx1 && cy0 <= cy1 && (cx1 - cx0 + 1) * (cy1 - cy0 + 1) <= 16) {
                  uint32_t near = 0xFFFFFFFFu;
                  for (int by = cy0; by <= cy1; ++by)
                    for (int bx = cx0; bx <= cx1; ++bx) near = min(near, tmin[by * nb + bx]);
                  valid = !(z_hi < near);
                }
              }
            }
          }
          const TriOwn<T> own = make_row_state<T>(valid, s, f, z_lo, x0, y0, x1, y1);
          if (!DRTK_DBG(dbg, 1)) {
            if (phase == 0) {
              raster_rows<T, TILE_SHIFT, false, FM, PEEL>(own, (cnt + 3) >> 2, x0, y0, zbuf, zthr, dbg);
            } else {
              raster_rows<T, TILE_SHIFT, true, FM, PEEL>(own, (cnt + 3) >> 2, x0, y0, zbuf, zthr, dbg);
            }
          }
        }
        if (tid == 0) DRTK_PHASE(2 + 4 * phase);
        if (kCoopMin > 0) {
          __syncthreads();
          const int ncoop = min(s_ncoop, kCoopMax);
          int t_here = tid;
          asm volatile("" : "+v"(t_here));
          const float x0f = static_cast<float>(x0), y0f = static_cast<float>(y0), first = static_cast<float>(t_here) + 0.5f;
          for (int b0 = 0; b0 < ncoop; b0 += kCoopBatch) {
            if (b0 > 0) __syncthreads();
            const int nb_here = min(kCoopBatch, ncoop - b0);
            constexpr int kPerWave = kCoopBatch / kRasterWaves;
            const int e = wave * kPerWave + lane;
            if (lane < kPerWave && e < nb_here) {
              const int f = s_coop[b0 + e];
              const uint4 pre = pre_n[f];
              TriSetup<T> s = {};
              const bool valid = tri_setup<T>(v_n, vi_n + int64_t(f) * 3, H, W, s);
              const TriRow<T> o = make_row_state<T>(valid, s, f, pre.z, x0, y0, x1, y1);
              uint32_t w[kTriWords];
              __builtin_memcpy(w, &o, sizeof(o));
#pragma unroll
              for (int j = 0; j < kTriWords; ++j) s_tri[e * kTriWords + j] = w[j];
            }
            __syncthreads();
            for (int i = 0; i < nb_here; ++i) {
              uint32_t w[kTriWords];
#pragma unroll
              for (int j = 0; j < kTriWords; ++j) w[j] = s_tri[i * kTriWords + j];
              TriRow<T> u;
              __builtin_memcpy(&u, w, sizeof(u));
              if (!DRTK_DBG(dbg, 1)) {
                if (phase == 0) {
                  shade_rows<T, TILE_SHIFT, false, FM, PEEL, kRasterBlock>(u, first, x0f, y0f, zbuf, zthr, dbg);
                } else {
                  shade_rows<T, TILE_SHIFT, true, FM, PEEL, kRasterBlock>(u, first, x0f, y0f, zbuf, zthr, dbg);
                }
              }
            }
          }
          if (ncoop > 0) {
            __syncthreads();
            if (tid == 0) s_ncoop = 0;
          }
        }
        if (phase == 1) break;
        __syncthreads();
        if (tid == 0) DRTK_PHASE(4);
        for (int by = wave; by < nb; by += kRasterWaves) {
          uint32_t m = 0;
          int l_here = lane;
          asm volatile("" : "+v"(l_here));
          if (lane < ss) {
#pragma unroll
            for (int r = 0; r < 8; ++r) m = max(m, static_cast<uint32_t>(zbuf[(((by << 3) + r) << TILE_SHIFT) + l_here] >> 32));
          }
          m = max(m, static_cast<uint32_t>(__builtin_amdgcn_mov_dpp(static_cast<int>(m), 0xB1, 0xF, 0xF, true)));
          m = max(m, static_cast<uint32_t>(__builtin_amdgcn_mov_dpp(static_cast<int>(m), 0x4E, 0xF, 0xF, true)));
          m = max(m, static_cast<uint32_t>(__builtin_amdgcn_mov_dpp(static_cast<int>(m), 0x141, 0xF, 0xF, true)));
          if ((lane & 7) == 0 && lane < ss) s_zmax[by * nb + (l_here >> 3)] = m;
        }
        __syncthreads();
        if (tid == 0) DRTK_PHASE(5);
      }
      __syncthreads();
      if (tid == 0) DRTK_PHASE(7);

      if (tid == 0) pop();
      for (int q = tid; q < rows * quads_per_row; q += kRasterBlock) {
        const int row = q / quads_per_row;
        const int col = (q - row * quads_per_row) << 2;
        const int y = y0 + row, x = x0 + col;
        if (x > x1) continue;
        int32_t idx4[4];
        float dep4[4];
        unsigned long long cleared = ~0ull;
        asm volatile("" : "+v"(cleared));
#pragma unroll
        for (int j = 0; j < 4; ++j) {
          const unsigned long long pv = zbuf[(row << TILE_SHIFT) + col + j];
          zbuf[(row << TILE_SHIFT) + col + j] = cleared;
          const uint32_t hi = static_cast<uint32_t>(pv >> 32);
          dep4[j] = (hi == 0xFFFFFFFFu) ? 0.0f : __uint_as_float(hi);
          idx4[j] = static_cast<int32_t>(static_cast<uint32_t>(pv & 0xFFFFFFFFu));
        }
        const int64_t o = img_base + int64_t(y) * W + x;
        if (vec_ok || x + 3 <= x1) {
          *reinterpret_cast<IQuad*>(index_img + o) = IQuad{idx4[0], idx4[1], idx4[2], idx4[3]};
          *reinterpret_cast<FQuad*>(depth_img + o) = FQuad{dep4[0], dep4[1], dep4[2], dep4[3]};
        } else {
#pragma unroll
          for (int j = 0; j < 4; ++j) {
            if (x + j <= x1) {
              index_img[o + j] = idx4[j];
              depth_img[o + j] = dep4[j];
            }
          }
        }
      }
    }
    if (tid == 0) DRTK_PHASE(8);
    __syncthreads();
    if (tid == 0) DRTK_PHASE(9);
  }
}

template <typename T, int TILE_SHIFT, bool FM>
__global__ __launch_bounds__(kRasterBlock, raster_waves_per_simd<T>()) void tile_raster_kernel(
    const T* __restrict__ v, const int32_t* __restrict__ vi, int F, int64_t V, int64_t vi_sN,
    int H, int W, int tiles_x, int tiles_per_view, const int32_t* __restrict__ tile_offset,
    const unsigned long long* __restrict__ tile_count, const float* __restrict__ view_stats,
    const int32_t* __restrict__ pairs, const int32_t* __restrict__ big_count,
    const int32_t* __restrict__ big_list, const uint2* __restrict__ tri_range, const uint4* __restrict__ tri_pre,
    const uint32_t* __restrict__ items, int32_t* __restrict__ queue, float* __restrict__ depth_img,
    int32_t* __restrict__ index_img, int dbg) {
  tile_raster_body<T, TILE_SHIFT, FM, kPlain>(
      v, vi, F, V, vi_sN, H, W, tiles_x, tiles_per_view, tile_offset, tile_count, view_stats, pairs, big_count, big_list,
      tri_range, tri_pre, items, queue, depth_img, index_img, dbg, 1, 0);
}

template <typename T, int TILE_SHIFT, bool FM, int MODE>
__global__ __launch_bounds__(kRasterBlock, (raster_waves_per_simd<T, MODE>())) void tile_raster_layer_kernel(
    const T* __restrict__ v, const int32_t* __restrict__ vi, int F, int64_t V, int64_t vi_sN,
    int H, int W, int tiles_x, int tiles_per_view, const int32_t* __restrict__ tile_offset,
    const unsigned long long* __restrict__ tile_count, const float* __restrict__ view_stats,
    const int32_t* __restrict__ pairs, const int32_t* __restrict__ big_count,
    const int32_t* __restrict__ big_list, const uint2* __restrict__ tri_range, const uint4* __restrict__ tri_pre,
    const uint32_t* __restrict__ items, int32_t* __restrict__ queue, float* __restrict__ depth_img,
    int32_t* __restrict__ index_img, int dbg, int num_layers, int layer) {
  static_assert(MODE == kLayerFirst || MODE == kLayerPeel, "the plain mode is tile_raster_kernel");
  tile_raster_body<T, TILE_SHIFT, FM, MODE>(
      v, vi, F, V, vi_sN, H, W, tiles_x, tiles_per_view, tile_offset, tile_count, view_stats, pairs, big_count, big_list,
      tri_range, tri_pre, items, queue, depth_img, index_img, dbg, num_layers, layer);
}

template <typename T>
__global__ __launch_bounds__(kBlock) void exact_div_selftest_kernel(
    unsigned long long seed, long long count, unsigned long long* __restrict__ mismatches) {
  const long long i = static_cast<long long>(blockIdx.x) * kBlock + threadIdx.x;
  unsigned long long local = 0;
  for (long long k = i; k < count; k += static_cast<long long>(gridDim.x) * kBlock) {
    unsigned long long z = seed + 0x9E3779B97F4A7C15ull * static_cast<unsigned long long>(k + 1);
    z = (z ^ (z >> 30)) * 0xBF58476D1CE4E5B9ull;
    z = (z ^ (z >> 27)) * 0x94D049BB133111EBull;
    z ^= z >> 31;
    unsigned long long w = z * 0xD6E8FEB86659FD93ull;
    w ^= w >> 32;
    T n, d;
    if constexpr (sizeof(T) == 4) {
      uint32_t md = static_cast<uint32_t>(z) & 0x7FFFFFu, mn = static_cast<uint32_t>(z >> 23) & 0x7FFFFFu;
      if ((k & 7) == 0) md = 0x7FFFFFu >> ((z >> 50) & 7);
      if ((k & 7) == 1) mn = 0x7FFFFFu << ((z >> 53) & 7) & 0x7FFFFFu;
      const int ed = 127 + static_cast<int>((w >> 8) % 81) - 40, en = ed - static_cast<int>((w >> 20) % 30);
      d = __uint_as_float((static_cast<uint32_t>(ed) << 23) | md);
      n = __uint_as_float((static_cast<uint32_t>(en > 1 ? en : 1) << 23) | mn);
    } else {
      unsigned long long md = z & 0xFFFFFFFFFFFFFull, mn = w & 0xFFFFFFFFFFFFFull;
      if ((k & 7) == 0) md = 0xFFFFFFFFFFFFFull >> ((z >> 55) & 15);
      const int ed = 1023 + static_cast<int>((w >> 52) % 81) - 40, en = ed - static_cast<int>((z >> 52) % 60);
      d = __longlong_as_double((static_cast<unsigned long long>(ed) << 52) | md);
      n = __longlong_as_double((static_cast<unsigned long long>(en) << 52) | mn);
    }
    const T r = T(1) / d;
    const T fast = exact_div(n, d, r, exact_div_ok(d));
    const T ref = n / d;
    if (!(fast == ref)) ++local;
    if (!(exact_rcp(d) == T(1) / d)) ++local;
    if constexpr (sizeof(T) == 4) {
      if (k < (1ll << 26)) {
        const int ex[8] = {127, 126, 128, 100, 160, 60, 190, 127 - 90};
        const float x = __uint_as_float((static_cast<uint32_t>(ex[k >> 23]) << 23) | static_cast<uint32_t>(k & 0x7FFFFF));
        if (!(exact_rcp(x) == 1.0f / x)) ++local;
        if (!(exact_rcp(-x) == 1.0f / -x)) ++local;
      }
    }
  }
  if (local) atomicAdd(mismatches, local);
}

template <typename T>
int rasterize_impl(
    const T* v, const int32_t* vi, int64_t N, int64_t V, int64_t F, int64_t vi_sN, int64_t H,
    int64_t W, float* depth_img, int32_t* index_img, void* workspace, size_t workspace_bytes,
    hipStream_t stream, int num_layers = 0) {
  const BinLayout L = make_layout(N, F, H, W);
  if (workspace_bytes < L.total_bytes) return DRTK_ERR_WORKSPACE_TOO_SMALL;
  if (N * H * W == 0) return DRTK_OK;
  if (num_layers == 1) num_layers = 0;
  char* ws = static_cast<char*>(workspace);
  auto* tile_count = reinterpret_cast<unsigned long long*>(ws + L.off_count);
  auto* tile_cursor = reinterpret_cast<unsigned long long*>(ws + L.off_cursor);
  auto* view_stats = reinterpret_cast<float*>(ws + L.off_view_stats);
  auto* big_count = reinterpret_cast<int32_t*>(ws + L.off_big_count);
  auto* tile_offset = reinterpret_cast<int32_t*>(ws + L.off_offset);
  auto* tri_range = reinterpret_cast<uint2*>(ws + L.off_range);
  auto* tri_pre = reinterpret_cast<uint4*>(ws + L.off_pre);
  auto* big_list = reinterpret_cast<int32_t*>(ws + L.off_big_list);
  auto* pairs = reinterpret_cast<int32_t*>(ws + L.off_pairs);
  auto* items = reinterpret_cast<uint32_t*>(ws + L.off_items);
  auto* queue = reinterpret_cast<int32_t*>(ws + L.off_queue);

  if (fill_bytes_async(ws, 0, L.zero_bytes, stream) != DRTK_OK) return DRTK_ERR_LAUNCH;
  const int64_t total = N * F;
  const dim3 tri_grid(static_cast<unsigned>(ceil_div(F > 0 ? F : 1, kBlock)), static_cast<unsigned>(N));
  if (total > 0) {
    DRTK_LAUNCH(
        bin_count_kernel<T>, tri_grid, dim3(kBlock), 0, stream, v, vi, (int)F, V, vi_sN, (int)H,
        (int)W, L.tile_shift, L.tiles_x, (int)L.tiles_per_view, tile_count, big_count, big_list,
        tri_range, tri_pre, view_stats);
    DRTK_RETURN_IF_LAUNCH_FAILED();
  }
  DRTK_LAUNCH(
      bin_scan_kernel, dim3(1), dim3(1024), 0, stream, tile_count, tile_offset, (int)L.num_tiles,
      L.tile_shift, split_threshold(N, F), items, queue);
  DRTK_RETURN_IF_LAUNCH_FAILED();
  if (total > 0) {
    DRTK_LAUNCH(
        bin_fill_kernel, tri_grid, dim3(kBlock), 0, stream, tri_range, (int)F, L.tiles_x,
        (int)L.tiles_per_view, tile_offset, tile_cursor, pairs);
    DRTK_RETURN_IF_LAUNCH_FAILED();
  }
#ifdef DRTK_RASTER_BLOCKS_PER_CU
  const int64_t resident = int64_t(num_compute_units()) * DRTK_RASTER_BLOCKS_PER_CU;
#else
  const int64_t resident = int64_t(num_compute_units()) * (raster_waves_per_simd<T>() / 2);
#endif
  const unsigned blocks = static_cast<unsigned>(std::min<int64_t>(L.max_items, resident));
#define DRTK_RASTER_LAUNCH(SHIFT, FM)                                                                              \
  DRTK_LAUNCH(                                                                                                    \
      (tile_raster_kernel<T, SHIFT, FM>), dim3(blocks), dim3(kRasterBlock), 0, stream, v, vi, (int)F, V, vi_sN,   \
      (int)H, (int)W, L.tiles_x, (int)L.tiles_per_view, tile_offset, tile_count, view_stats, pairs, big_count,    \
      big_list, tri_range, tri_pre, items, queue, depth_img, index_img, debug_flags())
  const bool fm = depth_order_setting() == DRTK_DEPTH_ORDER_FASTMATH;
  if (num_layers == 0) {
    if (L.tile_shift == 6) {
      if (fm) DRTK_RASTER_LAUNCH(6, true); else DRTK_RASTER_LAUNCH(6, false);
    } else {
      if (fm) DRTK_RASTER_LAUNCH(5, true); else DRTK_RASTER_LAUNCH(5, false);
    }
    DRTK_RETURN_IF_LAUNCH_FAILED();
    return DRTK_OK;
  }
#undef DRTK_RASTER_LAUNCH
  const unsigned peel_blocks =
      static_cast<unsigned>(std::min<int64_t>(L.max_items, int64_t(num_compute_units()) * (raster_waves_per_simd<T, kLayerPeel>() / 2)));
#define DRTK_LAYER_LAUNCH(SHIFT, FM, MODE, BLOCKS)                                                                 \
  DRTK_LAUNCH(                                                                                                    \
      (tile_raster_layer_kernel<T, SHIFT, FM, MODE>), dim3(BLOCKS), dim3(kRasterBlock), 0, stream, v, vi, (int)F, V, \
      vi_sN, (int)H, (int)W, L.tiles_x, (int)L.tiles_per_view, tile_offset, tile_count, view_stats, pairs, big_count, \
      big_list, tri_range, tri_pre, items, queue, depth_img, index_img, debug_flags(), num_layers, layer)
  for (int layer = 0; layer < num_layers; ++layer) {
    if (layer == 0) {
      if (L.tile_shift == 6) {
        if (fm) DRTK_LAYER_LAUNCH(6, true, kLayerFirst, blocks); else DRTK_LAYER_LAUNCH(6, false, kLayerFirst, blocks);
      } else {
        if (fm) DRTK_LAYER_LAUNCH(5, true, kLayerFirst, blocks); else DRTK_LAYER_LAUNCH(5, false, kLayerFirst, blocks);
      }
    } else {
      if (fill_bytes_async(queue + kQueueStride, 0, sizeof(int32_t) * kQueueStride * kQueueShards, stream) != DRTK_OK) return DRTK_ERR_LAUNCH;
      if (L.tile_shift == 6) {
        if (fm) DRTK_LAYER_LAUNCH(6, true, kLayerPeel, peel_blocks); else DRTK_LAYER_LAUNCH(6, false, kLayerPeel, peel_blocks);
      } else {
        if (fm) DRTK_LAYER_LAUNCH(5, true, kLayerPeel, peel_blocks); else DRTK_LAYER_LAUNCH(5, false, kLayerPeel, peel_blocks);
      }
    }
    DRTK_RETURN_IF_LAUNCH_FAILED();
  }
#undef DRTK_LAYER_LAUNCH
  return DRTK_OK;
}

}
}

namespace drtk_amd {
int rasterize_lines_dispatch(
    drtk_dtype_t dtype, const void* v, const int32_t* vi, int64_t N, int64_t V, int64_t F, int64_t vi_sN, int64_t H,
    int64_t W, float* depth_img, int32_t* index_img, void* workspace, size_t workspace_bytes, hipStream_t stream);
}
using namespace drtk_amd;

extern "C" int drtk_amd_rasterize_workspace_bytes(
    int64_t N, int64_t F, int64_t H, int64_t W, size_t* bytes) {
  if (!bytes || N < 0 || F < 0 || H <= 0 || W <= 0) return DRTK_ERR_INVALID_ARGUMENT;
  *bytes = make_layout(N, F, H, W).total_bytes;
  return DRTK_OK;
}

extern "C" int drtk_amd_rasterize(
    drtk_dtype_t dtype, const void* v, const int32_t* vi, int64_t N, int64_t V, int64_t F,
    int64_t vi_sN, int64_t H, int64_t W, int wireframe, float* depth_img, int32_t* index_img,
    void* workspace, size_t workspace_bytes, drtk_stream_t stream) {
  if (N < 0 || V < 0 || F < 0 || H <= 0 || W <= 0) return DRTK_ERR_INVALID_ARGUMENT;
  if (reinterpret_cast<uintptr_t>(workspace) % 16 != 0) return DRTK_ERR_INVALID_ARGUMENT;
  if (V >= 0x10000000LL) return DRTK_ERR_TOO_MANY_VERTICES;
  if (dtype != DRTK_F32 && dtype != DRTK_F64) return DRTK_ERR_INVALID_ARGUMENT;
  if (vi_sN != 0 && vi_sN != F * 3) return DRTK_ERR_INVALID_ARGUMENT;
  DRTK_FOR_VIEW_SLICES(N, n0, n, drtk_amd_rasterize(
      dtype, advance(v, n0 * V * 3, dtype_size(dtype)), advance_typed(vi, n0 * vi_sN), n, V, F, vi_sN, H, W, wireframe,
      advance_typed(depth_img, n0 * H * W), advance_typed(index_img, n0 * H * W), workspace, workspace_bytes, stream))
  if (wireframe) {
    if (N * H * W >= (int64_t(1) << 40)) return DRTK_ERR_INVALID_ARGUMENT;
    if (N * H * W > 0 && (!depth_img || !index_img)) return DRTK_ERR_INVALID_ARGUMENT;
  if (N * F > 0 && (!v || !vi)) return DRTK_ERR_INVALID_ARGUMENT;
    if (vi_sN != 0 && vi_sN != F * 3) return DRTK_ERR_INVALID_ARGUMENT;
    return rasterize_lines_dispatch(dtype, v, vi, N, V, F, vi_sN, H, W, depth_img, index_img, workspace, workspace_bytes, static_cast<hipStream_t>(stream));
  }
  if (H > 65535LL * 32 || W > 65535LL * 32 || N * F >= (int64_t(1) << 31) / kMaxSmallTiles ||
      N * H * W >= (int64_t(1) << 40))
    return DRTK_ERR_INVALID_ARGUMENT;
  if (N * H * W > 0 && (!depth_img || !index_img || !workspace)) return DRTK_ERR_INVALID_ARGUMENT;
  if (N * F > 0 && (!v || !vi)) return DRTK_ERR_INVALID_ARGUMENT;
  if (vi_sN != 0 && vi_sN != F * 3) return DRTK_ERR_INVALID_ARGUMENT;
  hipStream_t s = static_cast<hipStream_t>(stream);
  switch (dtype) {
    case DRTK_F32:
      return rasterize_impl<float>(static_cast<const float*>(v), vi, N, V, F, vi_sN, H, W, depth_img, index_img, workspace, workspace_bytes, s);
    case DRTK_F64:
      return rasterize_impl<double>(static_cast<const double*>(v), vi, N, V, F, vi_sN, H, W, depth_img, index_img, workspace, workspace_bytes, s);
    default:
      return DRTK_ERR_INVALID_ARGUMENT;
  }
}

extern "C" int drtk_amd_rasterize_layers_workspace_bytes(
    int64_t N, int64_t F, int64_t H, int64_t W, int num_layers, size_t* bytes) {
  if (!bytes || N < 0 || F < 0 || H <= 0 || W <= 0 || num_layers < 1 || num_layers > DRTK_AMD_MAX_RASTER_LAYERS) return DRTK_ERR_INVALID_ARGUMENT;
  *bytes = make_layout(N, F, H, W).total_bytes;
  return DRTK_OK;
}

extern "C" int drtk_amd_rasterize_layers(
    drtk_dtype_t dtype, const void* v, const int32_t* vi, int64_t N, int64_t V, int64_t F,
    int64_t vi_sN, int64_t H, int64_t W, int num_layers, float* depth_img, int32_t* index_img,
    void* workspace, size_t workspace_bytes, drtk_stream_t stream) {
  if (num_layers < 1 || num_layers > DRTK_AMD_MAX_RASTER_LAYERS) return DRTK_ERR_INVALID_ARGUMENT;
  if (N < 0 || V < 0 || F < 0 || H <= 0 || W <= 0) return DRTK_ERR_INVALID_ARGUMENT;
  if (reinterpret_cast<uintptr_t>(workspace) % 16 != 0) return DRTK_ERR_INVALID_ARGUMENT;
  if (V >= 0x10000000LL) return DRTK_ERR_TOO_MANY_VERTICES;
  if (dtype != DRTK_F32 && dtype != DRTK_F64) return DRTK_ERR_INVALID_ARGUMENT;
  if (vi_sN != 0 && vi_sN != F * 3) return DRTK_ERR_INVALID_ARGUMENT;
  const int64_t K = num_layers;
  DRTK_FOR_VIEW_SLICES(N, n0, n, drtk_amd_rasterize_layers(
      dtype, advance(v, n0 * V * 3, dtype_size(dtype)), advance_typed(vi, n0 * vi_sN), n, V, F, vi_sN, H, W, num_layers,
      advance_typed(depth_img, n0 * K * H * W), advance_typed(index_img, n0 * K * H * W), workspace, workspace_bytes, stream))
  if (H > 65535LL * 32 || W > 65535LL * 32 || N * F >= (int64_t(1) << 31) / kMaxSmallTiles ||
      N * K * H * W >= (int64_t(1) << 40))
    return DRTK_ERR_INVALID_ARGUMENT;
  if (N * H * W > 0 && (!depth_img || !index_img || !workspace)) return DRTK_ERR_INVALID_ARGUMENT;
  if (N * F > 0 && (!v || !vi)) return DRTK_ERR_INVALID_ARGUMENT;
  hipStream_t s = static_cast<hipStream_t>(stream);
  if (dtype == DRTK_F32)
    return rasterize_impl<float>(static_cast<const float*>(v), vi, N, V, F, vi_sN, H, W, depth_img, index_img, workspace, workspace_bytes, s, num_layers);
  return rasterize_impl<double>(static_cast<const double*>(v), vi, N, V, F, vi_sN, H, W, depth_img, index_img, workspace, workspace_bytes, s, num_layers);
}

extern "C" int drtk_amd_selftest_exact_div(
    drtk_dtype_t dtype, uint64_t seed, int64_t count, uint64_t* d_mismatches, drtk_stream_t stream) {
  if (!d_mismatches || count < 0) return DRTK_ERR_INVALID_ARGUMENT;
  hipStream_t s = static_cast<hipStream_t>(stream);
  if (fill_bytes_async(d_mismatches, 0, sizeof(uint64_t), s) != DRTK_OK) return DRTK_ERR_LAUNCH;
  const unsigned blocks = 4096;
  if (dtype == DRTK_F32) {
    DRTK_LAUNCH((exact_div_selftest_kernel<float>), dim3(blocks), dim3(kBlock), 0, s, seed, (long long)count, (unsigned long long*)d_mismatches);
  } else if (dtype == DRTK_F64) {
    DRTK_LAUNCH((exact_div_selftest_kernel<double>), dim3(blocks), dim3(kBlock), 0, s, seed, (long long)count, (unsigned long long*)d_mismatches);
  } else {
    return DRTK_ERR_INVALID_ARGUMENT;
  }
  DRTK_RETURN_IF_LAUNCH_FAILED();
  return DRTK_OK;
}
```

drtk_amd/csrc/torch_ops/rasterize.cpp:

```cpp
#include "common.hpp"

namespace {
using namespace drtk_amd_torch;

std::vector<Tensor> rasterize_hip(
    const Tensor& v, const Tensor& vi, int64_t height, int64_t width, bool wireframe) {
  TORCH_CHECK(v.defined() && vi.defined(), "rasterize(): expected all inputs to be defined");
  TORCH_CHECK(
      (v.device() == vi.device()) && v.is_cuda(),
      "rasterize(): expected all inputs to be on same cuda device");
  TORCH_CHECK(v.is_floating_point(), "rasterize(): expected v to have floating point type, but v has ", v.dtype());
  TORCH_CHECK(vi.dtype() == at::kInt, "rasterize(): expected vi to have int32 type, but vi has ", vi.dtype());
  TORCH_CHECK(
      v.layout() == at::kStrided && vi.layout() == at::kStrided,
      "rasterize(): expected all inputs to have torch.strided layout");
  TORCH_CHECK(
      (v.dim() == 3) && (vi.dim() == 3),
      "rasterize(): expected v.ndim == 3, vi.ndim == 3, but got v with sizes ", v.sizes(),
      " and vi with sizes ", vi.sizes());
  TORCH_CHECK(
      v.size(2) == 3 && vi.size(2) == 3,
      "rasterize(): expected third dim of v and last dim of vi to be 3, but got ", v.size(2), " and ", vi.size(2));
  TORCH_CHECK(
      vi.size(0) == v.size(0),
      "rasterize(): expected first dim of vi to match first dim of v, but got ", v.size(0), " and ", vi.size(0));
  TORCH_CHECK(
      v.size(1) < 0x10000000LL,
      "rasterize(): expected second dim of v to be less than 268435456, but got ", v.size(1));
  TORCH_CHECK(
      height > 0 && width > 0,
      "rasterize(): both height and width must be > 0, but got height: ", height, ", width: ", width);
  const drtk_dtype_t dt = dtype_of(v, "rasterize");

  c10::hip::OptionalHIPGuardMasqueradingAsCUDA guard(v.device());
  const auto v_c = v.contiguous();
  const ViArg via = prep_vi(vi);
  const int64_t N = v.size(0), V = v.size(1), F = vi.size(1);
  auto depth_img = out_empty({N, height, width}, v.options().dtype(at::kFloat));
  auto index_img = out_empty({N, height, width}, v.options().dtype(at::kInt));
  size_t ws_bytes = 0;
  check_status(
      wireframe ? drtk_amd_rasterize_lines_workspace_bytes(N, height, width, &ws_bytes)
                : drtk_amd_rasterize_workspace_bytes(N, F, height, width, &ws_bytes),
      "rasterize");
  auto ws = alloc_workspace(ws_bytes, v);
  check_status(
      drtk_amd_rasterize(
          dt, v_c.data_ptr(), via.ptr, N, V, F, via.sN, height, width, wireframe ? 1 : 0, depth_img.data_ptr<float>(),
          index_img.data_ptr<int32_t>(), ws.data_ptr(), ws_bytes, current_stream(v)),
      "rasterize");
  return {depth_img, index_img};
}

std::vector<Tensor> rasterize_cpu(const Tensor&, const Tensor&, int64_t, int64_t, bool) {
  no_cpu("rasterize");
}

tensor_list rasterize_op(const Tensor& v, const Tensor& vi, int64_t height, int64_t width, bool wireframe) {
  static auto op = c10::Dispatcher::singleton()
                       .findSchemaOrThrow("rasterize_ext::rasterize", "")
                       .typed<decltype(rasterize_op)>();
  return op.call(v, vi, height, width, wireframe);
}

tensor_list rasterize_autograd(const Tensor& v, const Tensor& vi, int64_t height, int64_t width, bool wireframe) {
  at::AutoDispatchBelowADInplaceOrView g;
  return rasterize_op(v, vi, height, width, wireframe);
}

tensor_list rasterize_autocast(const Tensor& v, const Tensor& vi, int64_t height, int64_t width, bool wireframe) {
  c10::impl::ExcludeDispatchKeyGuard no_autocast(c10::DispatchKey::Autocast);
  return rasterize_op(at::autocast::cached_cast(at::kFloat, v), vi, height, width, wireframe);
}

std::tuple<Tensor, Tensor> rasterize_layers_hip(
    const Tensor& v, const Tensor& vi, int64_t height, int64_t width, int64_t num_layers) {
  TORCH_CHECK(v.defined() && vi.defined(), "rasterize_layers(): expected all inputs to be defined");
  TORCH_CHECK(
      (v.device() == vi.device()) && v.is_cuda(),
      "rasterize_layers(): expected all inputs to be on same cuda device");
  TORCH_CHECK(v.is_floating_point(), "rasterize_layers(): expected v to have floating point type, but v has ", v.dtype());
  TORCH_CHECK(vi.dtype() == at::kInt, "rasterize_layers(): expected vi to have int32 type, but vi has ", vi.dtype());
  TORCH_CHECK(
      v.layout() == at::kStrided && vi.layout() == at::kStrided,
      "rasterize_layers(): expected all inputs to have torch.strided layout");
  TORCH_CHECK(
      (v.dim() == 3) && (vi.dim() == 3),
      "rasterize_layers(): expected v.ndim == 3, vi.ndim == 3, but got v with sizes ", v.sizes(),
      " and vi with sizes ", vi.sizes());
  TORCH_CHECK(
      v.size(2) == 3 && vi.size(2) == 3,
      "rasterize_layers(): expected third dim of v and last dim of vi to be 3, but got ", v.size(2), " and ", vi.size(2));
  TORCH_CHECK(
      vi.size(0) == v.size(0),
      "rasterize_layers(): expected first dim of vi to match first dim of v, but got ", v.size(0), " and ", vi.size(0));
  TORCH_CHECK(
      v.size(1) < 0x10000000LL,
      "rasterize_layers(): expected second dim of v to be less than 268435456, but got ", v.size(1));
  TORCH_CHECK(
      height > 0 && width > 0,
      "rasterize_layers(): both height and width must be > 0, but got height: ", height, ", width: ", width);
  TORCH_CHECK(
      num_layers >= 1 && num_layers <= DRTK_AMD_MAX_RASTER_LAYERS,
      "rasterize_layers(): num_layers must be in [1, ", DRTK_AMD_MAX_RASTER_LAYERS, "], but got ", num_layers);
  const drtk_dtype_t dt = dtype_of(v, "rasterize_layers");

  c10::hip::OptionalHIPGuardMasqueradingAsCUDA guard(v.device());
  const auto v_c = v.contiguous();
  const ViArg via = prep_vi(vi);
  const int64_t N = v.size(0), V = v.size(1), F = vi.size(1);
  const int K = static_cast<int>(num_layers);
  auto depth_img = out_empty({N, num_layers, height, width}, v.options().dtype(at::kFloat));
  auto index_img = out_empty({N, num_layers, height, width}, v.options().dtype(at::kInt));
  size_t ws_bytes = 0;
  check_status(drtk_amd_rasterize_layers_workspace_bytes(N, F, height, width, K, &ws_bytes), "rasterize_layers");
  auto ws = alloc_workspace(ws_bytes, v);
  check_status(
      drtk_amd_rasterize_layers(
          dt, v_c.data_ptr(), via.ptr, N, V, F, via.sN, height, width, K, depth_img.data_ptr<float>(),
          index_img.data_ptr<int32_t>(), ws.data_ptr(), ws_bytes, current_stream(v)),
      "rasterize_layers");
  return {depth_img, index_img};
}

std::tuple<Tensor, Tensor> rasterize_layers_cpu(const Tensor&, const Tensor&, int64_t, int64_t, int64_t) {
  no_cpu("rasterize_layers");
}

std::tuple<Tensor, Tensor> rasterize_layers_op(const Tensor& v, const Tensor& vi, int64_t height, int64_t width, int64_t num_layers) {
  static auto op = c10::Dispatcher::singleton()
                       .findSchemaOrThrow("drtk_amd_ext::rasterize_layers", "")
                       .typed<decltype(rasterize_layers_op)>();
  return op.call(v, vi, height, width, num_layers);
}

std::tuple<Tensor, Tensor> rasterize_layers_autograd(const Tensor& v, const Tensor& vi, int64_t height, int64_t width, int64_t num_layers) {
  at::AutoDispatchBelowADInplaceOrView g;
  return rasterize_layers_op(v, vi, height, width, num_layers);
}

std::tuple<Tensor, Tensor> rasterize_layers_autocast(const Tensor& v, const Tensor& vi, int64_t height, int64_t width, int64_t num_layers) {
  c10::impl::ExcludeDispatchKeyGuard no_autocast(c10::DispatchKey::Autocast);
  return rasterize_layers_op(at::autocast::cached_cast(at::kFloat, v), vi, height, width, num_layers);
}

}

TORCH_LIBRARY(rasterize_ext, m) {
  m.def("rasterize(Tensor v, Tensor vi, int height, int width, bool wireframe) -> Tensor[]");
}
TORCH_LIBRARY_IMPL(rasterize_ext, Autograd, m) {
  m.impl("rasterize", &rasterize_autograd);
}
TORCH_LIBRARY_IMPL(rasterize_ext, Autocast, m) {
  m.impl("rasterize", rasterize_autocast);
}
TORCH_LIBRARY_IMPL(rasterize_ext, CUDA, m) {
  m.impl("rasterize", &rasterize_hip);
}
TORCH_LIBRARY_IMPL(rasterize_ext, CPU, m) {
  m.impl("rasterize", &rasterize_cpu);
}

TORCH_LIBRARY_FRAGMENT(drtk_amd_ext, m) {
  m.def("rasterize_layers(Tensor v, Tensor vi, int height, int width, int num_layers) -> (Tensor, Tensor)");
}
TORCH_LIBRARY_IMPL(drtk_amd_ext, Autograd, m) {
  m.impl("rasterize_layers", &rasterize_layers_autograd);
}
TORCH_LIBRARY_IMPL(drtk_amd_ext, Autocast, m) {
  m.impl("rasterize_layers", rasterize_layers_autocast);
}
TORCH_LIBRARY_IMPL(drtk_amd_ext, CUDA, m) {
  m.impl("rasterize_layers", &rasterize_layers_hip);
}
TORCH_LIBRARY_IMPL(drtk_amd_ext, CPU, m) {
  m.impl("rasterize_layers", &rasterize_layers_cpu);
}
```

drtk_amd/rasterize.py:

```python
import ctypes
from typing import Tuple

import torch as th
from drtk_amd.utils import load_torch_ops
from drtk_amd.utils.load_torch_ops import native_library_paths

load_torch_ops("drtk.rasterize_ext")

_DEPTH_ORDERS = {"strict": 0, "fastmath": 1}


def set_depth_order(order: str) -> None:
    if order not in _DEPTH_ORDERS:
        raise ValueError(f"depth order must be one of {sorted(_DEPTH_ORDERS)}, got {order!r}")
    status = ctypes.CDLL(native_library_paths()[0]).drtk_amd_set_depth_order(_DEPTH_ORDERS[order])
    if status != 0:
        raise RuntimeError(f"drtk_amd_set_depth_order: status {status}")


def get_depth_order() -> str:
    o = ctypes.CDLL(native_library_paths()[0]).drtk_amd_get_depth_order()
    return next(k for k, v in _DEPTH_ORDERS.items() if v == o)


def _batched_vi(vi: th.Tensor, n: int) -> th.Tensor:
    return vi[None].expand(n, -1, -1) if vi.ndim == 2 else vi


@th.compiler.disable
def rasterize(
    v: th.Tensor,
    vi: th.Tensor,
    height: int,
    width: int,
    wireframe: bool = False,
) -> th.Tensor:
    _, index_img = th.ops.rasterize_ext.rasterize(v, _batched_vi(vi, v.shape[0]), height, width, wireframe)
    return index_img


@th.compiler.disable
def rasterize_with_depth(
    v: th.Tensor,
    vi: th.Tensor,
    height: int,
    width: int,
    wireframe: bool = False,
) -> Tuple[th.Tensor, th.Tensor]:
    depth_img, index_img = th.ops.rasterize_ext.rasterize(
        v, _batched_vi(vi, v.shape[0]), height, width, wireframe
    )
    return depth_img, index_img


MAX_RASTER_LAYERS = 8


@th.compiler.disable
def rasterize_layers(
    v: th.Tensor,
    vi: th.Tensor,
    height: int,
    width: int,
    num_layers: int,
) -> th.Tensor:
    _, index_img = th.ops.drtk_amd_ext.rasterize_layers(v, _batched_vi(vi, v.shape[0]), height, width, num_layers)
    return index_img


@th.compiler.disable
def rasterize_layers_with_depth(
    v: th.Tensor,
    vi: th.Tensor,
    height: int,
    width: int,
    num_layers: int,
) -> Tuple[th.Tensor, th.Tensor]:
    depth_img, index_img = th.ops.drtk_amd_ext.rasterize_layers(
        v, _batched_vi(vi, v.shape[0]), height, width, num_layers
    )
    return depth_img, index_img
```

include/drtk_amd.h:

```cpp
#ifndef DRTK_AMD_H
#define DRTK_AMD_H

#include <stddef.h>
#include <stdint.h>

#ifdef __cplusplus
extern "C" {
#endif

#if defined(__GNUC__) || defined(__clang__)
#pragma GCC visibility push(default)
#endif

#define DRTK_AMD_VERSION_MAJOR 0
#define DRTK_AMD_VERSION_MINOR 4

typedef enum { DRTK_F32 = 0, DRTK_F64 = 1 } drtk_dtype_t;

typedef enum {
  DRTK_OK = 0,
  DRTK_ERR_INVALID_ARGUMENT = -1,
  DRTK_ERR_WORKSPACE_TOO_SMALL = -2,
  DRTK_ERR_LAUNCH = -3,
  DRTK_ERR_UNSUPPORTED = -4,
  DRTK_ERR_TOO_MANY_VERTICES = -5
} drtk_status_t;

typedef void* drtk_stream_t;

const char* drtk_amd_status_string(int status);
const char* drtk_amd_version(void);

typedef enum {
  DRTK_DEPTH_ORDER_STRICT = 0,
  DRTK_DEPTH_ORDER_FASTMATH = 1
} drtk_depth_order_t;
int drtk_amd_set_depth_order(int order);
int drtk_amd_get_depth_order(void);
int drtk_amd_rasterize_workspace_bytes(int64_t N, int64_t F, int64_t H, int64_t W, size_t* bytes);
int drtk_amd_rasterize_lines_workspace_bytes(int64_t N, int64_t H, int64_t W, size_t* bytes);
int drtk_amd_rasterize(
    drtk_dtype_t dtype, const void* v, const int32_t* vi, int64_t N, int64_t V, int64_t F,
    int64_t vi_sN, int64_t H, int64_t W, int wireframe, float* depth_img, int32_t* index_img,
    void* workspace, size_t workspace_bytes, drtk_stream_t stream);

#define DRTK_AMD_MAX_RASTER_LAYERS 8
int drtk_amd_rasterize_layers_workspace_bytes(int64_t N, int64_t F, int64_t H, int64_t W, int num_layers, size_t* bytes);
int drtk_amd_rasterize_layers(
    drtk_dtype_t dtype, const void* v, const int32_t* vi, int64_t N, int64_t V, int64_t F,
    int64_t vi_sN, int64_t H, int64_t W, int num_layers, float* depth_img, int32_t* index_img,
    void* workspace, size_t workspace_bytes, drtk_stream_t stream);

int drtk_amd_render(
    drtk_dtype_t dtype, const void* v, const int32_t* vi, const int32_t* index_img, int64_t N,
    int64_t V, int64_t F, int64_t vi_sN, int64_t H, int64_t W, void* depth_img, void* bary_img,
    drtk_stream_t stream);

int drtk_amd_render_backward(
    drtk_dtype_t dtype, const void* v, const int32_t* vi, const int32_t* index_img,
    const void* grad_depth_img, const void* grad_bary_img, int64_t N, int64_t V, int64_t F,
    int64_t vi_sN, int64_t H, int64_t W, void* grad_v, drtk_stream_t stream);

int drtk_amd_interpolate(
    drtk_dtype_t dtype, const void* attrs, const int32_t* vi, const int32_t* index_img,
    const void* bary_img, int64_t N, int64_t V, int64_t C, int64_t F, int64_t vi_sN, int64_t H,
    int64_t W, void* out, drtk_stream_t stream);

int drtk_amd_interpolate_masked(
    drtk_dtype_t dtype, const void* attrs, const int32_t* vi, const int32_t* index_img,
    const void* bary_img, int64_t N, int64_t V, int64_t C, int64_t F, int64_t vi_sN, int64_t H,
    int64_t W, void* out, drtk_stream_t stream);

int drtk_amd_interpolate_backward(
    drtk_dtype_t dtype, const void* grad_out, const void* attrs, const int32_t* vi,
    const int32_t* index_img, const void* bary_img, int64_t N, int64_t V, int64_t C, int64_t F,
    int64_t vi_sN, int64_t H, int64_t W, void* attr_grad, void* bary_grad, drtk_stream_t stream);
int drtk_amd_interpolate_backward_workspace_bytes(drtk_dtype_t dtype, int64_t N, int64_t V, int64_t C, size_t* bytes);
int drtk_amd_interpolate_backward_ws(
    drtk_dtype_t dtype, const void* grad_out, const void* attrs, const int32_t* vi,
    const int32_t* index_img, const void* bary_img, int64_t N, int64_t V, int64_t C, int64_t F,
    int64_t vi_sN, int64_t H, int64_t W, void* attr_grad, void* bary_grad, void* workspace, size_t workspace_bytes,
    drtk_stream_t stream);

int drtk_amd_edge_grad_backward_workspace_bytes(
    drtk_dtype_t dtype, int64_t N, int64_t H, int64_t W, size_t* bytes);
int drtk_amd_edge_grad_backward(
    drtk_dtype_t dtype, const void* v_pix, const void* img, const int32_t* index_img,
    const int32_t* vi, const void* grad_output, int64_t N, int64_t V, int64_t C, int64_t F,
    int64_t vi_sN, int64_t H, int64_t W, double max_dp_dr, void* grad_v_pix_img, void* workspace,
    size_t workspace_bytes, drtk_stream_t stream);

int drtk_amd_edge_grad_backward_fused_workspace_bytes(
    drtk_dtype_t dtype, int64_t N, int64_t H, int64_t W, size_t* bytes);
int drtk_amd_edge_grad_backward_fused(
    drtk_dtype_t dtype, const void* v_pix, const void* img, const int32_t* index_img,
    const int32_t* vi, const void* bary_img, const void* grad_output, int64_t N, int64_t V, int64_t C,
    int64_t F, int64_t vi_sN, int64_t H, int64_t W, double max_dp_dr, void* grad_v_pix,
    void* workspace, size_t workspace_bytes, drtk_stream_t stream);

int drtk_amd_interpolation_matrix(
    drtk_dtype_t dtype, const int32_t* vi, const int32_t* index_img, const void* bary_img,
    const int64_t* row_pixels, int64_t R, int64_t N, int64_t F, int64_t vi_sN, int64_t H, int64_t W,
    int64_t* col_indices, void* values, drtk_stream_t stream);
int drtk_amd_interpolation_matrix_backward(
    drtk_dtype_t dtype, const void* grad_values, const int32_t* vi, const int32_t* index_img,
    const int64_t* row_pixels, int64_t R, int64_t N, int64_t F, int64_t vi_sN, int64_t H, int64_t W,
    void* bary_grad, drtk_stream_t stream);
int drtk_amd_interpolation_normal_matrix_values(
    drtk_dtype_t dtype, const int32_t* pair_indices, const int32_t* index_img, const void* bary_img,
    int64_t N, int64_t F, int64_t pair_sN, int64_t H, int64_t W, int64_t nnz, void* values,
    drtk_stream_t stream);
int drtk_amd_interpolation_normal_matrix_values_backward(
    drtk_dtype_t dtype, const void* grad_values, const int32_t* pair_indices, const int32_t* index_img,
    const void* bary_img, int64_t N, int64_t F, int64_t pair_sN, int64_t H, int64_t W, void* bary_grad,
    drtk_stream_t stream);

int drtk_amd_mipmap_grid_sampler_2d(
    drtk_dtype_t dtype, const void* const* levels, const int64_t* level_h, const int64_t* level_w,
    const int64_t* level_sN, int mipmaps, const void* grid, const int64_t* grid_layout, const void* vt_dxdy_img, int64_t N,
    int64_t C, int64_t H, int64_t W, int max_aniso, int padding_mode, int interpolation_mode, int align_corners,
    int force_max_aniso, int clip_grad, void* out, drtk_stream_t stream);
int drtk_amd_mipmap_grid_sampler_2d_backward(
    drtk_dtype_t dtype, const void* grad_out, const void* const* levels, const int64_t* level_h,
    const int64_t* level_w, const int64_t* level_sN, int mipmaps, const void* grid, const int64_t* grid_layout,
    const void* vt_dxdy_img, int64_t N, int64_t C, int64_t H, int64_t W, int max_aniso, int padding_mode,
    int interpolation_mode, int align_corners, int force_max_aniso, int clip_grad, void* const* grad_levels,
    void* grad_grid, const int64_t* grad_grid_layout, drtk_stream_t stream);

int drtk_amd_grid_scatter_2d(
    drtk_dtype_t dtype, const void* input, const void* grid, const int64_t* grid_layout, int64_t N, int64_t C, int64_t H,
    int64_t W, int64_t output_height, int64_t output_width, int padding_mode, int interpolation_mode, int align_corners,
    void* out, uint32_t* route_counts, drtk_stream_t stream);
int drtk_amd_grid_scatter_2d_backward(
    drtk_dtype_t dtype, const void* grad_out, const void* input, const void* grid, const int64_t* grid_layout, int64_t N,
    int64_t C, int64_t H, int64_t W, int64_t output_height, int64_t output_width, int padding_mode, int interpolation_mode,
    int align_corners, void* grad_input, void* grad_grid, const int64_t* grad_grid_layout, drtk_stream_t stream);

int drtk_amd_screen_space_uv_derivative(
    drtk_dtype_t dtype, const void* v, int64_t v_sN, const void* vt, int64_t vt_sN, const int32_t* vi,
    const int32_t* vti, const int32_t* index_img, const void* bary_img, const uint8_t* mask,
    const void* campos, const void* camrot, const void* focal, int64_t N, int64_t V, int64_t T, int64_t F,
    int64_t H, int64_t W, void* out, drtk_stream_t stream);

int drtk_amd_transform_pinhole(
    drtk_dtype_t dtype, const void* v, int64_t v_sN, const void* campos, const void* camrot,
    const void* focal, const void* princpt, int64_t N, int64_t V, void* v_pix, void* v_cam,
    drtk_stream_t stream);
int drtk_amd_transform_pinhole_backward(
    drtk_dtype_t dtype, const void* v, int64_t v_sN, const void* campos, const void* camrot,
    const void* focal, const void* princpt, const void* grad_v_pix, int64_t N, int64_t V,
    void* grad_v, drtk_stream_t stream);

#define DRTK_GEOMETRY_CHUNK 256
int drtk_amd_geometry_face_forward(
    drtk_dtype_t dtype, const void* v, int64_t v_sN, const int32_t* vi, int64_t vi_sN, const void* vt, int64_t vt_sN,
    const int32_t* vti, int64_t N, int64_t V, int64_t T, int64_t F, void* normals, void* areas, void* edges,
    void* dpdt, void* dpdt_u, void* v012, drtk_stream_t stream);
int drtk_amd_geometry_face_backward(
    drtk_dtype_t dtype, const void* v, int64_t v_sN, const int32_t* vi, int64_t vi_sN, const void* vt, int64_t vt_sN,
    const int32_t* vti, int64_t N, int64_t V, int64_t T, int64_t F, const void* grad_vert, const void* vert_sums,
    const void* grad_normals, const void* grad_areas, const void* grad_edges, const void* grad_dpdt,
    const void* grad_v012, void* pos_rows, void* uv_rows, drtk_stream_t stream);
int drtk_amd_geometry_face_gather(
    drtk_dtype_t dtype, const void* grad_vert, const void* vert_sums, const int32_t* vi, int64_t vi_sN, int64_t N,
    int64_t V, int64_t F, int64_t A, void* out, drtk_stream_t stream);
int drtk_amd_geometry_vertex_gather_workspace_bytes(
    drtk_dtype_t dtype, int64_t N, int64_t B, int64_t num_chunks, int64_t A, size_t* bytes);
int drtk_amd_geometry_vertex_gather(
    drtk_dtype_t dtype, const void* src, int64_t src_sN, int per_corner, int64_t A, const int32_t* crow,
    const int32_t* entries, const int32_t* chunk_ptr, const int32_t* chunk_begin, const int32_t* chunk_row,
    int64_t num_chunks, int64_t B, int64_t N, int64_t V, int64_t F, int normalize, void* out, void* vert_sums,
    void* workspace, size_t workspace_bytes, drtk_stream_t stream);

int drtk_amd_selftest_exact_div(
    drtk_dtype_t dtype, uint64_t seed, int64_t count, uint64_t* d_mismatches, drtk_stream_t stream);

int drtk_amd_kernel_timing_begin(void);
int drtk_amd_kernel_timing_report(char* buf, size_t capacity, size_t* needed);

#if defined(__GNUC__) || defined(__clang__)
#pragma GCC visibility pop
#endif

#ifdef __cplusplus
}
#endif
#endif
```

Baseline: 6483 Mpix/s.

## Add index-only rasterize path, batch binning per thread, multi-block tile scan

Adds a rasterize_index entry point that skips writing the depth image when the caller only needs triangle indices, and routes the non-wireframe Python rasterize() to it. This removes N*H*W float stores per view. The binning kernels now process two triangles per thread and hoist the vertex loads ahead of the bbox math to expose more memory-level parallelism. The tile scan kernel moves from a single 1024-thread block to multiple 256-thread blocks, each recomputing global prefix totals redundantly. The change spans several kernels and adds a new API surface, so grid launch sizes must match the new per-thread triangle count.

```diff
diff --git a/drtk_amd/capi.py b/drtk_amd/capi.py
--- a/drtk_amd/capi.py
+++ b/drtk_amd/capi.py
@@ -104,6 +104,7 @@
     "drtk_amd_rasterize_workspace_bytes",
     "drtk_amd_rasterize_lines_workspace_bytes",
     "drtk_amd_rasterize",
+    "drtk_amd_rasterize_index",
     "drtk_amd_rasterize_layers_workspace_bytes",
     "drtk_amd_rasterize_layers",
     "drtk_amd_render",
@@ -244,6 +245,26 @@
     return depth, index
 
 
+@_on_tensor_device
+def rasterize_index(v, vi, height, width, stream=None, workspace=None, out=None) -> th.Tensor:
+    v = v.contiguous()
+    N, V, _ = v.shape
+    vi_c, vi_sN, F = _vi(vi, N)
+    if out is not None:
+        index = out
+        assert index.shape == (N, height, width) and index.is_contiguous() and index.dtype == th.int32
+    else:
+        index = _out(N, height, width, dtype=th.int32, device=v.device)
+    nbytes = rasterize_workspace_bytes(N, F, height, width)
+    ws = workspace if workspace is not None else _out(nbytes, dtype=th.uint8, device=v.device)
+    _check(
+        lib().drtk_amd_rasterize_index(
+            ctypes.c_int(_dt(v)), _p(v), _p(vi_c), _i(N), _i(V), _i(F), _i(vi_sN), _i(height), _i(width),
+            _p(index), _p(ws), ctypes.c_size_t(ws.numel()), _stream(v, stream)),
+        "rasterize_index")
+    return index
+
+
 MAX_RASTER_LAYERS = 8
 
 
diff --git a/drtk_amd/csrc/rasterize.hip b/drtk_amd/csrc/rasterize.hip
--- a/drtk_amd/csrc/rasterize.hip
+++ b/drtk_amd/csrc/rasterize.hip
@@ -160,15 +160,12 @@
 
 template <typename T>
 __device__ __forceinline__ bool tri_bbox(
-    const T* __restrict__ v_n, const int32_t* __restrict__ vi_face, int H, int W, int& bx0,
+    const int32_t (&vtx)[3], const T (&p)[9], int H, int W, int& bx0,
     int& by0, int& bx1, int& by1, bool& positive, float& z_mean, uint32_t& z_lo_bits) {
-  const int32_t vi_0 = static_cast<int32_t>(static_cast<uint32_t>(vi_face[0]) & 0x0FFFFFFFu);
-  const int32_t vi_1 = vi_face[1];
-  const int32_t vi_2 = vi_face[2];
-  if (vi_0 == vi_1 && vi_1 == vi_2) return false;
-  const T p0x = v_n[3 * (int64_t)vi_0 + 0], p0y = v_n[3 * (int64_t)vi_0 + 1], p0z = v_n[3 * (int64_t)vi_0 + 2];
-  const T p1x = v_n[3 * (int64_t)vi_1 + 0], p1y = v_n[3 * (int64_t)vi_1 + 1], p1z = v_n[3 * (int64_t)vi_1 + 2];
-  const T p2x = v_n[3 * (int64_t)vi_2 + 0], p2y = v_n[3 * (int64_t)vi_2 + 1], p2z = v_n[3 * (int64_t)vi_2 + 2];
+  if (vtx[0] == vtx[1] && vtx[1] == vtx[2]) return false;
+  const T p0x = p[0], p0y = p[1], p0z = p[2];
+  const T p1x = p[3], p1y = p[4], p1z = p[5];
+  const T p2x = p[6], p2y = p[7], p2z = p[8];
   if (!(p0z > T(1e-8f) && p1z > T(1e-8f) && p2z > T(1e-8f))) return false;
   const T min_x = min3(p0x, p1x, p2x), min_y = min3(p0y, p1y, p2y);
   const T max_x = max3(p0x, p1x, p2x), max_y = max3(p0y, p1y, p2y);
@@ -362,6 +359,10 @@
   return pos;
 }
 
+#ifndef DRTK_BIN_TRIS
+#define DRTK_BIN_TRIS 2
+#endif
+constexpr int kBinTris = DRTK_BIN_TRIS;
 template <typename T>
 __global__ __launch_bounds__(kBlock) void bin_count_kernel(
     const T* __restrict__ v, const int32_t* __restrict__ vi, int F, int64_t V, int64_t vi_sN, int H,
@@ -369,74 +370,101 @@
     int32_t* __restrict__ big_count, int32_t* __restrict__ big_list,
     uint2* __restrict__ tri_range, uint4* __restrict__ tri_pre, float* __restrict__ view_stats) {
   const int n = blockIdx.y;
-  const int f = blockIdx.x * kBlock + threadIdx.x;
-  const bool in_range = f < F;
-  int bx0, by0, bx1, by1;
-  uint2 r = make_uint2(kCulled, kCulled);
-  int tx0 = 0, ty0 = 0, tw = 0, ntiles = 0;
-  bool positive = false;
-  float z_mean = 0.0f;
-  uint32_t z_lo_bits = 0;
-  if (in_range &&
-      tri_bbox<T>(v + int64_t(n) * V * 3, vi + int64_t(n) * vi_sN + int64_t(f) * 3, H, W, bx0, by0, bx1, by1, positive, z_mean, z_lo_bits)) {
-    const bool fits = bx1 < 65536 && by1 < 65536;
-    tri_pre[int64_t(n) * F + f] = make_uint4(
-        static_cast<uint32_t>(bx0) | (static_cast<uint32_t>(bx1) << 16), static_cast<uint32_t>(by0) | (static_cast<uint32_t>(by1) << 16),
-        fits ? z_lo_bits : 0u, fits ? 1u : 0u);
-    tx0 = bx0 >> tile_shift;
-    ty0 = by0 >> tile_shift;
-    const int tx1 = bx1 >> tile_shift, ty1 = by1 >> tile_shift;
-    r.x = static_cast<uint32_t>(tx0) | (static_cast<uint32_t>(tx1) << 16);
-    r.y = static_cast<uint32_t>(ty0) | (static_cast<uint32_t>(ty1) << 16) | (positive ? kFacingBit : 0u);
-    tw = tx1 - tx0 + 1;
-    ntiles = tw * (ty1 - ty0 + 1);
-  }
-  if ((blockIdx.x & 63) == 0) {
-    const bool live = ntiles >= 1;
-    float zp = (live && positive) ? z_mean : 0.0f, zn = (live && !positive) ? z_mean : 0.0f;
-#pragma unroll
-    for (int o = 32; o > 0; o >>= 1) {
-      zp += __shfl_xor(zp, o);
-      zn += __shfl_xor(zn, o);
-    }
-    const int cp = __popcll(__ballot(live && positive)), cn = __popcll(__ballot(live && !positive));
-    if (lane_id() == 0 && (cp | cn)) {
-      float* st = view_stats + 4 * n;
-      if (cp) {
-        atomic_add_global(st + 0, zp);
-        atomic_add_global(st + 1, static_cast<float>(cp));
+  const T* v_n = v + int64_t(n) * V * 3;
+  const int32_t* vi_n = vi + int64_t(n) * vi_sN;
+  const int f0 = blockIdx.x * (kBlock * kBinTris) + threadIdx.x;
+  int32_t vtx[kBinTris][3];
+  T p[kBinTris][9];
+#pragma unroll
+  for (int j = 0; j < kBinTris; ++j) {
+    const int32_t* face = vi_n + int64_t(min(f0 + j * kBlock, F - 1)) * 3;
+    vtx[j][0] = static_cast<int32_t>(static_cast<uint32_t>(face[0]) & 0x0FFFFFFFu);
+    vtx[j][1] = face[1];
+    vtx[j][2] = face[2];
+  }
+#pragma unroll
+  for (int j = 0; j < kBinTris; ++j) {
+    const bool degenerate = vtx[j][0] == vtx[j][1] && vtx[j][1] == vtx[j][2];
+#pragma unroll
+    for (int k = 0; k < 3; ++k) {
+      const T* vert = v_n + 3 * (int64_t)(degenerate ? 0 : vtx[j][k]);
+#pragma unroll
+      for (int c = 0; c < 3; ++c) p[j][3 * k + c] = vert[c];
+    }
+  }
+#pragma unroll
+  for (int j = 0; j < kBinTris; ++j) {
+    const int f = f0 + j * kBlock;
+    const bool in_range = f < F;
+    int bx0, by0, bx1, by1;
+    uint2 r = make_uint2(kCulled, kCulled);
+    int tx0 = 0, ty0 = 0, tw = 0, ntiles = 0;
+    bool positive = false;
+    float z_mean = 0.0f;
+    uint32_t z_lo_bits = 0;
+    if (in_range && tri_bbox<T>(vtx[j], p[j], H, W, bx0, by0, bx1, by1, positive, z_mean, z_lo_bits)) {
+      const bool fits = bx1 < 65536 && by1 < 65536;
+      tri_pre[int64_t(n) * F + f] = make_uint4(
+          static_cast<uint32_t>(bx0) | (static_cast<uint32_t>(bx1) << 16), static_cast<uint32_t>(by0) | (static_cast<uint32_t>(by1) << 16),
+          fits ? z_lo_bits : 0u, fits ? 1u : 0u);
+      tx0 = bx0 >> tile_shift;
+      ty0 = by0 >> tile_shift;
+      const int tx1 = bx1 >> tile_shift, ty1 = by1 >> tile_shift;
+      r.x = static_cast<uint32_t>(tx0) | (static_cast<uint32_t>(tx1) << 16);
+      r.y = static_cast<uint32_t>(ty0) | (static_cast<uint32_t>(ty1) << 16) | (positive ? kFacingBit : 0u);
+      tw = tx1 - tx0 + 1;
+      ntiles = tw * (ty1 - ty0 + 1);
+    }
+    if ((blockIdx.x & 63) == 0) {
+      const bool live = ntiles >= 1;
+      float zp = (live && positive) ? z_mean : 0.0f, zn = (live && !positive) ? z_mean : 0.0f;
+#pragma unroll
+      for (int o = 32; o > 0; o >>= 1) {
+        zp += __shfl_xor(zp, o);
+        zn += __shfl_xor(zn, o);
       }
-      if (cn) {
-        atomic_add_global(st + 2, zn);
-        atomic_add_global(st + 3, static_cast<float>(cn));
+      const int cp = __popcll(__ballot(live && positive)), cn = __popcll(__ballot(live && !positive));
+      if (lane_id() == 0 && (cp | cn)) {
+        float* st = view_stats + 4 * n;
+        if (cp) {
+          atomic_add_global(st + 0, zp);
+          atomic_add_global(st + 1, static_cast<float>(cp));
+        }
+        if (cn) {
+          atomic_add_global(st + 2, zn);
+          atomic_add_global(st + 3, static_cast<float>(cn));
+        }
       }
     }
-  }
-  if (in_range) tri_range[int64_t(n) * F + f] = r;
-  const bool small = ntiles >= 1 && ntiles <= kMaxSmallTiles;
-  const int base = n * tiles_per_view;
-  for (int s = 0; s < kMaxSmallTiles; ++s) {
-    const bool on = small && s < ntiles;
-    const int dy = on ? s / tw : 0;
-    const int dx = on ? s - dy * tw : 0;
-    const int t = base + (ty0 + dy) * tiles_x + tx0 + dx;
-    wave_agg_inc2<true, false>(tile_count, t, on, positive);
-  }
-  const bool big = ntiles > kMaxSmallTiles;
-  if (__ballot(big)) {
-    const int pos = wave_agg_inc<true>(big_count, n, big);
-    if (big) big_list[int64_t(n) * F + pos] = f;
-  }
-}
-
-__global__ __launch_bounds__(1024) void bin_scan_kernel(
+    if (in_range) tri_range[int64_t(n) * F + f] = r;
+    const bool small = ntiles >= 1 && ntiles <= kMaxSmallTiles;
+    const int base = n * tiles_per_view;
+    for (int s = 0; s < kMaxSmallTiles; ++s) {
+      const bool on = small && s < ntiles;
+      const int dy = on ? s / tw : 0;
+      const int dx = on ? s - dy * tw : 0;
+      const int t = base + (ty0 + dy) * tiles_x + tx0 + dx;
+      wave_agg_inc2<true, false>(tile_count, t, on, positive);
+    }
+    const bool big = ntiles > kMaxSmallTiles;
+    if (__ballot(big)) {
+      const int pos = wave_agg_inc<true>(big_count, n, big);
+      if (big) big_list[int64_t(n) * F + pos] = f;
+    }
+  }
+}
+
+constexpr int kScanThreads = 256, kScanMaxBlocks = 64;
+__global__ __launch_bounds__(kScanThreads) void bin_scan_kernel(
     const unsigned long long* __restrict__ tile_count64, int32_t* __restrict__ tile_offset, int num_tiles,
     int tile_shift, int split4, uint32_t* __restrict__ items, int32_t* __restrict__ queue) {
-  constexpr int kThreads = 1024, kWaves = kThreads / kWave, kVals = 5, kReg = 8;
+  constexpr int kThreads = kScanThreads, kWaves = kThreads / kWave, kVals = 5, kReg = 8;
   __shared__ int32_t s_wave[kWaves][kVals];
+  __shared__ int32_t s_all[kWaves][2 * kVals];
   const int tid = threadIdx.x, lane = tid & (kWave - 1), wave = tid / kWave;
-  const int chunk = (num_tiles + kThreads - 1) / kThreads;
-  const int begin = tid * chunk;
+  const int chunk = (num_tiles + static_cast<int>(gridDim.x) * kThreads - 1) / (static_cast<int>(gridDim.x) * kThreads);
+  const int block_begin = min(static_cast<int>(blockIdx.x) * kThreads * chunk, num_tiles);
+  const int begin = min((static_cast<int>(blockIdx.x) * kThreads + tid) * chunk, num_tiles);
   const int end = min(begin + chunk, num_tiles);
   const int max_split_log = max(0, min(2, tile_shift - 4));
   auto split_log_of = [&](int c) {
@@ -444,32 +472,44 @@
     return min(sl, max_split_log);
   };
   auto class_of = [&](int c, int sl) { return c == 0 ? 3 : 2 - sl; };
+  auto count_of = [&](int i) -> int32_t { return static_cast<int32_t>(tile_count64[i] & 0xFFFFFFFFull); };
+  auto tally = [&](int32_t (&v)[kVals], int c) {
+    const int sl = split_log_of(c);
+    const int cls = class_of(c, sl);
+    v[0] += c;
+#pragma unroll
+    for (int k = 0; k < 4; ++k) v[1 + k] += cls == k ? 1 << (2 * sl) : 0;
+  };
   const bool in_regs = chunk <= kReg;
   int32_t cnt[kReg];
 #pragma unroll
-  for (int j = 0; j < kReg; ++j) {
-    cnt[j] = (in_regs && begin + j < end) ? static_cast<int32_t>(tile_count64[begin + j] & 0xFFFFFFFFull) : 0;
-  }
-  auto count_at = [&](int j) -> int32_t {
-    return static_cast<int32_t>(tile_count64[begin + j] & 0xFFFFFFFFull);
-  };
+  for (int j = 0; j < kReg; ++j) cnt[j] = (in_regs && begin + j < end) ? count_of(begin + j) : 0;
+  int32_t acc[kVals] = {0, 0, 0, 0, 0}, bef[kVals];
+  int i = tid;
+#pragma unroll 8
+  for (; i < block_begin; i += kThreads) tally(acc, count_of(i));
+#pragma unroll
+  for (int k = 0; k < kVals; ++k) bef[k] = acc[k];
+#pragma unroll 8
+  for (; i < num_tiles; i += kThreads) tally(acc, count_of(i));
   int32_t v[kVals] = {0, 0, 0, 0, 0};
-  auto tally = [&](int c) {
-    const int sl = split_log_of(c);
-    v[0] += c;
-    v[1 + class_of(c, sl)] += 1 << (2 * sl);
-  };
   if (in_regs) {
 #pragma unroll
     for (int j = 0; j < kReg; ++j) {
-      if (begin + j < end) tally(cnt[j]);
+      if (begin + j < end) tally(v, cnt[j]);
     }
   } else {
-    for (int j = 0; begin + j < end; ++j) tally(count_at(j));
+    for (int j = 0; begin + j < end; ++j) tally(v, count_of(begin + j));
   }
   int32_t inc[kVals];
 #pragma unroll
   for (int k = 0; k < kVals; ++k) {
+    int32_t b = bef[k], a = acc[k];
+#pragma unroll
+    for (int o = kWave / 2; o > 0; o >>= 1) {
+      b += __shfl_xor(b, o);
+      a += __shfl_xor(a, o);
+    }
     int32_t x = v[k];
 #pragma unroll
     for (int o = 1; o < kWave; o <<= 1) {
@@ -478,41 +518,43 @@
     }
     inc[k] = x;
     if (lane == kWave - 1) s_wave[wave][k] = x;
+    if (lane == 0) s_all[wave][k] = b, s_all[wave][kVals + k] = a;
   }
   __syncthreads();
   int32_t before[kVals], total[kVals];
 #pragma unroll
   for (int k = 0; k < kVals; ++k) {
-    int32_t lo = 0, all = 0;
+    int32_t lo = 0, b = 0, a = 0;
+#pragma unroll
     for (int w = 0; w < kWaves; ++w) {
-      const int32_t t = s_wave[w][k];
-      all += t;
-      if (w < wave) lo += t;
-    }
-    before[k] = lo + inc[k] - v[k];
-    total[k] = all;
+      if (w < wave) lo += s_wave[w][k];
+      b += s_all[w][k];
+      a += s_all[w][kVals + k];
+    }
+    before[k] = b + lo + inc[k] - v[k];
+    total[k] = a;
   }
   int32_t slot[4];
   {
-    int32_t acc = 0;
+    int32_t acc_items = 0;
 #pragma unroll
     for (int k = 0; k < 4; ++k) {
-      slot[k] = acc + before[1 + k];
-      acc += total[1 + k];
-    }
-    if (tid == 0) {
-      queue[1] = acc;
+      slot[k] = acc_items + before[1 + k];
+      acc_items += total[1 + k];
+    }
+    if (blockIdx.x == 0 && tid == 0) {
+      queue[1] = acc_items;
       tile_offset[num_tiles] = total[0];
     }
   }
   int32_t run = before[0];
-  auto emit = [&](int i, int c) {
-    tile_offset[i] = run;
+  auto emit = [&](int t, int c) {
+    tile_offset[t] = run;
     run += c;
     const int sl = split_log_of(c);
     const int cls = class_of(c, sl);
     const int n_sub = 1 << (2 * sl);
-    for (int j = 0; j < n_sub; ++j) items[slot[cls] + j] = make_item(static_cast<uint32_t>(i), j, sl) | (c == 0 ? kItemEmpty : 0u);
+    for (int j = 0; j < n_sub; ++j) items[slot[cls] + j] = make_item(static_cast<uint32_t>(t), j, sl) | (c == 0 ? kItemEmpty : 0u);
     slot[cls] += n_sub;
   };
   if (in_regs) {
@@ -521,7 +563,7 @@
       if (begin + j < end) emit(begin + j, cnt[j]);
     }
   } else {
-    for (int j = 0; begin + j < end; ++j) emit(begin + j, count_at(j));
+    for (int j = 0; begin + j < end; ++j) emit(begin + j, count_of(begin + j));
   }
 }
 
@@ -530,11 +572,20 @@
     const int32_t* __restrict__ tile_offset, unsigned long long* __restrict__ tile_cursor,
     int32_t* __restrict__ pairs) {
   const int n = blockIdx.y;
-  const int f = blockIdx.x * kBlock + threadIdx.x;
+  const int f0 = blockIdx.x * (kBlock * kBinTris) + threadIdx.x;
+  uint2 rr[kBinTris];
+#pragma unroll
+  for (int j = 0; j < kBinTris; ++j) {
+    const int f = f0 + j * kBlock;
+    rr[j] = f < F ? tri_range[int64_t(n) * F + f] : make_uint2(kCulled, kCulled);
+  }
+#pragma unroll
+  for (int j = 0; j < kBinTris; ++j) {
+  const int f = f0 + j * kBlock;
   int tx0 = 0, ty0 = 0, tw = 0, ntiles = 0;
   bool positive = false;
-  if (f < F) {
-    const uint2 r = tri_range[int64_t(n) * F + f];
+  {
+    const uint2 r = rr[j];
     if (r.x != kCulled) {
       tx0 = r.x & 0xFFFF;
       ty0 = r.y & 0xFFFF;
@@ -585,6 +636,7 @@
       const int pos = static_cast<int>(positive ? lo : hi) + rank_[s];
       pairs[positive ? tile_offset[t_[s]] + pos : tile_offset[t_[s] + 1] - 1 - pos] = f;
     }
+  }
   }
 }
 
@@ -802,7 +854,7 @@
 constexpr int kCoopBatch = 64;
 constexpr int kCoopMax = 256;
 
-template <typename T, int TILE_SHIFT, bool FM, int MODE>
+template <typename T, int TILE_SHIFT, bool FM, int MODE, bool WRITE_DEPTH = true>
 __device__ __forceinline__ void tile_raster_body(
     const T* __restrict__ v, const int32_t* __restrict__ vi, int F, int64_t V, int64_t vi_sN,
     int H, int W, int tiles_x, int tiles_per_view, const int32_t* __restrict__ tile_offset,
@@ -814,6 +866,7 @@
   constexpr int TILE = 1 << TILE_SHIFT;
   constexpr int NPIX = TILE * TILE;
   constexpr bool PEEL = MODE == kLayerPeel;
+  static_assert(WRITE_DEPTH || MODE == kPlain, "the layer kernels read the previous layer's depth_img");
   __shared__ unsigned long long zbuf[NPIX];
   unsigned long long* zthr = nullptr;
   uint32_t* tmin = nullptr;
@@ -961,11 +1014,11 @@
           asm volatile("" : "+v"(none), "+v"(zero));
           if (vec_ok || x + 3 <= x1) {
             *reinterpret_cast<IQuad*>(index_img + o) = IQuad{none, none, none, none};
-            *reinterpret_cast<FQuad*>(depth_img + o) = FQuad{zero, zero, zero, zero};
+            if constexpr (WRITE_DEPTH) *reinterpret_cast<FQuad*>(depth_img + o) = FQuad{zero, zero, zero, zero};
           } else {
             for (int j = 0; j < 4 && x + j <= x1; ++j) {
               index_img[o + j] = none;
-              depth_img[o + j] = zero;
+              if constexpr (WRITE_DEPTH) depth_img[o + j] = zero;
             }
           }
         }
@@ -1206,19 +1259,19 @@
           const unsigned long long pv = zbuf[(row << TILE_SHIFT) + col + j];
           zbuf[(row << TILE_SHIFT) + col + j] = cleared;
           const uint32_t hi = static_cast<uint32_t>(pv >> 32);
-          dep4[j] = (hi == 0xFFFFFFFFu) ? 0.0f : __uint_as_float(hi);
+          dep4[j] = (WRITE_DEPTH && hi != 0xFFFFFFFFu) ? __uint_as_float(hi) : 0.0f;
           idx4[j] = static_cast<int32_t>(static_cast<uint32_t>(pv & 0xFFFFFFFFu));
         }
         const int64_t o = img_base + int64_t(y) * W + x;
         if (vec_ok || x + 3 <= x1) {
           *reinterpret_cast<IQuad*>(index_img + o) = IQuad{idx4[0], idx4[1], idx4[2], idx4[3]};
-          *reinterpret_cast<FQuad*>(depth_img + o) = FQuad{dep4[0], dep4[1], dep4[2], dep4[3]};
+          if constexpr (WRITE_DEPTH) *reinterpret_cast<FQuad*>(depth_img + o) = FQuad{dep4[0], dep4[1], dep4[2], dep4[3]};
         } else {
 #pragma unroll
           for (int j = 0; j < 4; ++j) {
             if (x + j <= x1) {
               index_img[o + j] = idx4[j];
-              depth_img[o + j] = dep4[j];
+              if constexpr (WRITE_DEPTH) depth_img[o + j] = dep4[j];
             }
           }
         }
@@ -1230,7 +1283,7 @@
   }
 }
 
-template <typename T, int TILE_SHIFT, bool FM>
+template <typename T, int TILE_SHIFT, bool FM, bool WRITE_DEPTH>
 __global__ __launch_bounds__(kRasterBlock, raster_waves_per_simd<T>()) void tile_raster_kernel(
     const T* __restrict__ v, const int32_t* __restrict__ vi, int F, int64_t V, int64_t vi_sN,
     int H, int W, int tiles_x, int tiles_per_view, const int32_t* __restrict__ tile_offset,
@@ -1239,7 +1292,7 @@
     const int32_t* __restrict__ big_list, const uint2* __restrict__ tri_range, const uint4* __restrict__ tri_pre,
     const uint32_t* __restrict__ items, int32_t* __restrict__ queue, float* __restrict__ depth_img,
     int32_t* __restrict__ index_img, int dbg) {
-  tile_raster_body<T, TILE_SHIFT, FM, kPlain>(
+  tile_raster_body<T, TILE_SHIFT, FM, kPlain, WRITE_DEPTH>(
       v, vi, F, V, vi_sN, H, W, tiles_x, tiles_per_view, tile_offset, tile_count, view_stats, pairs, big_count, big_list,
       tri_range, tri_pre, items, queue, depth_img, index_img, dbg, 1, 0);
 }
@@ -1326,8 +1379,8 @@
   auto* queue = reinterpret_cast<int32_t*>(ws + L.off_queue);
 
   if (fill_bytes_async(ws, 0, L.zero_bytes, stream) != DRTK_OK) return DRTK_ERR_LAUNCH;
-  const int64_t total = N * F;
-  const dim3 tri_grid(static_cast<unsigned>(ceil_div(F > 0 ? F : 1, kBlock)), static_cast<unsigned>(N));
+  const int64_t total = V > 0 ? N * F : 0;
+  const dim3 tri_grid(static_cast<unsigned>(ceil_div(F > 0 ? F : 1, kBlock * kBinTris)), static_cast<unsigned>(N));
   if (total > 0) {
     DRTK_LAUNCH(
         bin_count_kernel<T>, tri_grid, dim3(kBlock), 0, stream, v, vi, (int)F, V, vi_sN, (int)H,
@@ -1335,8 +1388,9 @@
         tri_range, tri_pre, view_stats);
     DRTK_RETURN_IF_LAUNCH_FAILED();
   }
+  const unsigned scan_blocks = static_cast<unsigned>(std::min<int64_t>(kScanMaxBlocks, std::max<int64_t>(1, ceil_div(L.num_tiles, kScanThreads))));
   DRTK_LAUNCH(
-      bin_scan_kernel, dim3(1), dim3(1024), 0, stream, tile_count, tile_offset, (int)L.num_tiles,
+      bin_scan_kernel, dim3(scan_blocks), dim3(kScanThreads), 0, stream, tile_count, tile_offset, (int)L.num_tiles,
       L.tile_shift, split_threshold(N, F), items, queue);
   DRTK_RETURN_IF_LAUNCH_FAILED();
   if (total > 0) {
@@ -1351,21 +1405,26 @@
   const int64_t resident = int64_t(num_compute_units()) * (raster_waves_per_simd<T>() / 2);
 #endif
   const unsigned blocks = static_cast<unsigned>(std::min<int64_t>(L.max_items, resident));
-#define DRTK_RASTER_LAUNCH(SHIFT, FM)                                                                              \
+#define DRTK_RASTER_LAUNCH(SHIFT, FM, WRITE_DEPTH)                                                                 \
   DRTK_LAUNCH(                                                                                                    \
-      (tile_raster_kernel<T, SHIFT, FM>), dim3(blocks), dim3(kRasterBlock), 0, stream, v, vi, (int)F, V, vi_sN,   \
-      (int)H, (int)W, L.tiles_x, (int)L.tiles_per_view, tile_offset, tile_count, view_stats, pairs, big_count,    \
+      (tile_raster_kernel<T, SHIFT, FM, WRITE_DEPTH>), dim3(blocks), dim3(kRasterBlock), 0, stream, v, vi, (int)F, V, \
+      vi_sN, (int)H, (int)W, L.tiles_x, (int)L.tiles_per_view, tile_offset, tile_count, view_stats, pairs, big_count, \
       big_list, tri_range, tri_pre, items, queue, depth_img, index_img, debug_flags())
+#define DRTK_RASTER_LAUNCH_FM(SHIFT, WRITE_DEPTH)                                                   \
+  do {                                                                                              \
+    if (fm) DRTK_RASTER_LAUNCH(SHIFT, true, WRITE_DEPTH); else DRTK_RASTER_LAUNCH(SHIFT, false, WRITE_DEPTH); \
+  } while (0)
   const bool fm = depth_order_setting() == DRTK_DEPTH_ORDER_FASTMATH;
   if (num_layers == 0) {
     if (L.tile_shift == 6) {
-      if (fm) DRTK_RASTER_LAUNCH(6, true); else DRTK_RASTER_LAUNCH(6, false);
+      if (depth_img) DRTK_RASTER_LAUNCH_FM(6, true); else DRTK_RASTER_LAUNCH_FM(6, false);
     } else {
-      if (fm) DRTK_RASTER_LAUNCH(5, true); else DRTK_RASTER_LAUNCH(5, false);
+      if (depth_img) DRTK_RASTER_LAUNCH_FM(5, true); else DRTK_RASTER_LAUNCH_FM(5, false);
     }
     DRTK_RETURN_IF_LAUNCH_FAILED();
     return DRTK_OK;
   }
+#undef DRTK_RASTER_LAUNCH_FM
 #undef DRTK_RASTER_LAUNCH
   const unsigned peel_blocks =
       static_cast<unsigned>(std::min<int64_t>(L.max_items, int64_t(num_compute_units()) * (raster_waves_per_simd<T, kLayerPeel>() / 2)));
@@ -1446,6 +1505,29 @@
     default:
       return DRTK_ERR_INVALID_ARGUMENT;
   }
+}
+
+extern "C" int drtk_amd_rasterize_index(
+    drtk_dtype_t dtype, const void* v, const int32_t* vi, int64_t N, int64_t V, int64_t F,
+    int64_t vi_sN, int64_t H, int64_t W, int32_t* index_img, void* workspace, size_t workspace_bytes,
+    drtk_stream_t stream) {
+  if (N < 0 || V < 0 || F < 0 || H <= 0 || W <= 0) return DRTK_ERR_INVALID_ARGUMENT;
+  if (reinterpret_cast<uintptr_t>(workspace) % 16 != 0) return DRTK_ERR_INVALID_ARGUMENT;
+  if (V >= 0x10000000LL) return DRTK_ERR_TOO_MANY_VERTICES;
+  if (dtype != DRTK_F32 && dtype != DRTK_F64) return DRTK_ERR_INVALID_ARGUMENT;
+  if (vi_sN != 0 && vi_sN != F * 3) return DRTK_ERR_INVALID_ARGUMENT;
+  DRTK_FOR_VIEW_SLICES(N, n0, n, drtk_amd_rasterize_index(
+      dtype, advance(v, n0 * V * 3, dtype_size(dtype)), advance_typed(vi, n0 * vi_sN), n, V, F, vi_sN, H, W,
+      advance_typed(index_img, n0 * H * W), workspace, workspace_bytes, stream))
+  if (H > 65535LL * 32 || W > 65535LL * 32 || N * F >= (int64_t(1) << 31) / kMaxSmallTiles ||
+      N * H * W >= (int64_t(1) << 40))
+    return DRTK_ERR_INVALID_ARGUMENT;
+  if (N * H * W > 0 && (!index_img || !workspace)) return DRTK_ERR_INVALID_ARGUMENT;
+  if (N * F > 0 && (!v || !vi)) return DRTK_ERR_INVALID_ARGUMENT;
+  hipStream_t s = static_cast<hipStream_t>(stream);
+  if (dtype == DRTK_F32)
+    return rasterize_impl<float>(static_cast<const float*>(v), vi, N, V, F, vi_sN, H, W, nullptr, index_img, workspace, workspace_bytes, s);
+  return rasterize_impl<double>(static_cast<const double*>(v), vi, N, V, F, vi_sN, H, W, nullptr, index_img, workspace, workspace_bytes, s);
 }
 
 extern "C" int drtk_amd_rasterize_layers_workspace_bytes(
diff --git a/drtk_amd/csrc/torch_ops/rasterize.cpp b/drtk_amd/csrc/torch_ops/rasterize.cpp
--- a/drtk_amd/csrc/torch_ops/rasterize.cpp
+++ b/drtk_amd/csrc/torch_ops/rasterize.cpp
@@ -71,6 +71,71 @@
 tensor_list rasterize_autocast(const Tensor& v, const Tensor& vi, int64_t height, int64_t width, bool wireframe) {
   c10::impl::ExcludeDispatchKeyGuard no_autocast(c10::DispatchKey::Autocast);
   return rasterize_op(at::autocast::cached_cast(at::kFloat, v), vi, height, width, wireframe);
+}
+
+Tensor rasterize_index_hip(const Tensor& v, const Tensor& vi, int64_t height, int64_t width) {
+  TORCH_CHECK(v.defined() && vi.defined(), "rasterize(): expected all inputs to be defined");
+  TORCH_CHECK(
+      (v.device() == vi.device()) && v.is_cuda(),
+      "rasterize(): expected all inputs to be on same cuda device");
+  TORCH_CHECK(v.is_floating_point(), "rasterize(): expected v to have floating point type, but v has ", v.dtype());
+  TORCH_CHECK(vi.dtype() == at::kInt, "rasterize(): expected vi to have int32 type, but vi has ", vi.dtype());
+  TORCH_CHECK(
+      v.layout() == at::kStrided && vi.layout() == at::kStrided,
+      "rasterize(): expected all inputs to have torch.strided layout");
+  TORCH_CHECK(
+      (v.dim() == 3) && (vi.dim() == 3),
+      "rasterize(): expected v.ndim == 3, vi.ndim == 3, but got v with sizes ", v.sizes(),
+      " and vi with sizes ", vi.sizes());
+  TORCH_CHECK(
+      v.size(2) == 3 && vi.size(2) == 3,
+      "rasterize(): expected third dim of v and last dim of vi to be 3, but got ", v.size(2), " and ", vi.size(2));
+  TORCH_CHECK(
+      vi.size(0) == v.size(0),
+      "rasterize(): expected first dim of vi to match first dim of v, but got ", v.size(0), " and ", vi.size(0));
+  TORCH_CHECK(
+      v.size(1) < 0x10000000LL,
+      "rasterize(): expected second dim of v to be less than 268435456, but got ", v.size(1));
+  TORCH_CHECK(
+      height > 0 && width > 0,
+      "rasterize(): both height and width must be > 0, but got height: ", height, ", width: ", width);
+  const drtk_dtype_t dt = dtype_of(v, "rasterize");
+
+  c10::hip::OptionalHIPGuardMasqueradingAsCUDA guard(v.device());
+  const auto v_c = v.contiguous();
+  const ViArg via = prep_vi(vi);
+  const int64_t N = v.size(0), V = v.size(1), F = vi.size(1);
+  auto index_img = out_empty({N, height, width}, v.options().dtype(at::kInt));
+  size_t ws_bytes = 0;
+  check_status(drtk_amd_rasterize_workspace_bytes(N, F, height, width, &ws_bytes), "rasterize");
+  auto ws = alloc_workspace(ws_bytes, v);
+  check_status(
+      drtk_amd_rasterize_index(
+          dt, v_c.data_ptr(), via.ptr, N, V, F, via.sN, height, width, index_img.data_ptr<int32_t>(), ws.data_ptr(),
+          ws_bytes, current_stream(v)),
+      "rasterize");
+  return index_img;
+}
+
+Tensor rasterize_index_cpu(const Tensor&, const Tensor&, int64_t, int64_t) {
+  no_cpu("rasterize");
+}
+
+Tensor rasterize_index_op(const Tensor& v, const Tensor& vi, int64_t height, int64_t width) {
+  static auto op = c10::Dispatcher::singleton()
+                       .findSchemaOrThrow("drtk_amd_ext::rasterize_index", "")
+                       .typed<decltype(rasterize_index_op)>();
+  return op.call(v, vi, height, width);
+}
+
+Tensor rasterize_index_autograd(const Tensor& v, const Tensor& vi, int64_t height, int64_t width) {
+  at::AutoDispatchBelowADInplaceOrView g;
+  return rasterize_index_op(v, vi, height, width);
+}
+
+Tensor rasterize_index_autocast(const Tensor& v, const Tensor& vi, int64_t height, int64_t width) {
+  c10::impl::ExcludeDispatchKeyGuard no_autocast(c10::DispatchKey::Autocast);
+  return rasterize_index_op(at::autocast::cached_cast(at::kFloat, v), vi, height, width);
 }
 
 std::tuple<Tensor, Tensor> rasterize_layers_hip(
@@ -164,16 +229,21 @@
 
 TORCH_LIBRARY_FRAGMENT(drtk_amd_ext, m) {
   m.def("rasterize_layers(Tensor v, Tensor vi, int height, int width, int num_layers) -> (Tensor, Tensor)");
+  m.def("rasterize_index(Tensor v, Tensor vi, int height, int width) -> Tensor");
 }
 TORCH_LIBRARY_IMPL(drtk_amd_ext, Autograd, m) {
   m.impl("rasterize_layers", &rasterize_layers_autograd);
+  m.impl("rasterize_index", &rasterize_index_autograd);
 }
 TORCH_LIBRARY_IMPL(drtk_amd_ext, Autocast, m) {
   m.impl("rasterize_layers", rasterize_layers_autocast);
+  m.impl("rasterize_index", rasterize_index_autocast);
 }
 TORCH_LIBRARY_IMPL(drtk_amd_ext, CUDA, m) {
   m.impl("rasterize_layers", &rasterize_layers_hip);
+  m.impl("rasterize_index", &rasterize_index_hip);
 }
 TORCH_LIBRARY_IMPL(drtk_amd_ext, CPU, m) {
   m.impl("rasterize_layers", &rasterize_layers_cpu);
-}
+  m.impl("rasterize_index", &rasterize_index_cpu);
+}
diff --git a/drtk_amd/rasterize.py b/drtk_amd/rasterize.py
--- a/drtk_amd/rasterize.py
+++ b/drtk_amd/rasterize.py
@@ -35,6 +35,8 @@
     width: int,
     wireframe: bool = False,
 ) -> th.Tensor:
+    if not wireframe:
+        return th.ops.drtk_amd_ext.rasterize_index(v, _batched_vi(vi, v.shape[0]), height, width)
     _, index_img = th.ops.rasterize_ext.rasterize(v, _batched_vi(vi, v.shape[0]), height, width, wireframe)
     return index_img
 
diff --git a/include/drtk_amd.h b/include/drtk_amd.h
--- a/include/drtk_amd.h
+++ b/include/drtk_amd.h
@@ -43,6 +43,10 @@
     drtk_dtype_t dtype, const void* v, const int32_t* vi, int64_t N, int64_t V, int64_t F,
     int64_t vi_sN, int64_t H, int64_t W, int wireframe, float* depth_img, int32_t* index_img,
     void* workspace, size_t workspace_bytes, drtk_stream_t stream);
+int drtk_amd_rasterize_index(
+    drtk_dtype_t dtype, const void* v, const int32_t* vi, int64_t N, int64_t V, int64_t F,
+    int64_t vi_sN, int64_t H, int64_t W, int32_t* index_img, void* workspace, size_t workspace_bytes,
+    drtk_stream_t stream);
 
 #define DRTK_AMD_MAX_RASTER_LAYERS 8
 int drtk_amd_rasterize_layers_workspace_bytes(int64_t N, int64_t F, int64_t H, int64_t W, int num_layers, size_t* bytes);
```

After: 6554 Mpix/s (median of 2 runs). Within noise of the previous version (+1.1%).
